# aakhundov/tf-attend-infer-repeat

Measured on AMD Instinct MI355X. Metric: images/sec AIR train step, 50x50 multi-MNIST b=64 N=3, higher is better.
Workload: dtype bf16; 1 GPU; configs[1]: AIR train step, 50x50 canvas, 0-2 objects, batch 64/GPU, 3 steps, 256 LSTM, z=50 (training.py:100-122); global_batch=64, hipgraph=True, steps_per_graph_replay=20, graph_mode=one hipGraph replay = 20 train steps, parallelism=dp1, backward=reference, phase=single order

## Files before the change

include/air_hip.h:

```cpp
#ifndef AIR_HIP_H
#define AIR_HIP_H

#include <stdint.h>

#ifdef __cplusplus
extern "C" {
#endif

#define AIR_ABI_VERSION 6

#define AIR_EINVAL   (-1)
#define AIR_ELIMIT   (-2)
#define AIR_EALIGN   (-3)

int air_abi_version(void);
const char* air_strerror(int code);

enum {
    AIR_DYN_PRIOR_LOG_ODDS = 0,
    AIR_DYN_TEMPERATURE    = 1,
    AIR_DYN_STOP_THRESHOLD = 2,
    AIR_DYN_LEARNING_RATE  = 3,
    AIR_DYN_CLIP_NORM      = 4,
    AIR_DYN_SCALE_PM = 5, AIR_DYN_SCALE_PV = 6,
    AIR_DYN_SHIFT_PM = 7, AIR_DYN_SHIFT_PV = 8,
    AIR_DYN_VAE_PM   = 9, AIR_DYN_VAE_PV   = 10,
    AIR_DYN_LIK_STD  = 11,
    AIR_DYN_GRAD_SCALE = 12,
    AIR_DYN_SCALE_PLV = 13, AIR_DYN_SHIFT_PLV = 14, AIR_DYN_VAE_PLV = 15,
    AIR_DYN_COUNT    = 16
};

enum {
    AIR_IST_GLOBAL_STEP = 0,
    AIR_IST_COUNT = 4
};

typedef struct {
    int32_t slot;
    int32_t flags;
    float init, iters, factor, vmin, vmax;
} air_schedule_t;

enum {
    AIR_ATT_S = 0, AIR_ATT_X = 1, AIR_ATT_Y = 2,
    AIR_ATT_ZPRE = 3,
    AIR_ATT_Z = 4,
    AIR_ATT_ZPROB = 5,
    AIR_ATT_KL_Z = 6, AIR_ATT_KL_SCALE = 7, AIR_ATT_KL_SHIFT = 8, AIR_ATT_KL_VAE = 9,
    AIR_ATT_MASK_PREV = 10,
    AIR_ATT_MASK = 11,
    AIR_ATT_ST_BACK = 12,
    AIR_ATT_STRIDE = 16
};
#define AIR_OUT_STRIDE 8

enum {
    AIR_ACT_NONE = 0, AIR_ACT_RELU = 1, AIR_ACT_SOFTPLUS = 2,
    AIR_ACT_SIGMOID_NOISE = 3
};
enum {
    AIR_GRAD_NONE = 0,
    AIR_GRAD_RELU = 1,
    AIR_GRAD_SOFTPLUS = 2
};
enum {
    AIR_EPI_GENERIC = 0,
    AIR_EPI_LSTM_FWD = 1,
    AIR_EPI_REPARAM_FWD = 2,
    AIR_EPI_LSTM_BWD = 3,
    AIR_EPI_REPARAM_BWD = 4,
    AIR_EPI_LSTM_BWD_TAIL = 5,
    AIR_EPI_LSTM_FWD0 = 6
};
typedef struct {
    const air_schedule_t* sched ; int32_t nsched; float* dyn; const int32_t* istate;
    float* normals; int64_t n_normal; float* uniforms; int64_t n_uniform; uint64_t seed;
    const float* twin_src; uint16_t* twin_dst; int64_t twin_n;
} air_step_job_t;
typedef struct {
    const float* A; const float* B; float* C;
    int32_t M, N, K, lda, ldb, ldc;
    int32_t transA, transB;
    const float* bias;
    const float* addend; int32_t ldadd;
    const float* aux;    int32_t ldaux;
    float   aux_scale;
    int32_t act;
    int32_t actgrad;
    int32_t accumulate;
    int32_t precision;
    int32_t epi;
    int32_t tile_m, tile_n;
    int32_t ksplit;
    int32_t addend_slabs;
    int32_t i0;
    const float* p0; const float* p1; const float* p2; const float* p3;
    float* q0; float* q1; float* q2;
    const air_step_job_t* step_job;
    const uint16_t* A16; const uint16_t* B16;
    uint16_t* C16; uint16_t* q0_16; uint16_t* q2_16;
    const uint16_t* B16p;
} air_gemm_t;
int air_gemm_slabs(int K, int ksplit);
int air_gemm(const air_gemm_t* g, void* stream);
int air_gemm_kernel_name(const air_gemm_t* g, char* buf, int n);

int air_bf16_twin(const float* src, uint16_t* dst, int64_t n, void* stream);

typedef struct {
    int64_t src_off, dst_off;
    int32_t K, N, gates, exclusive;
} air_panel_t;
#define AIR_MAX_PANELS 16
int air_panel_shadow(const float* params, uint16_t* panel_shadow, const air_panel_t* panels ,
                     int count, void* stream);

typedef struct {
    const float* A; const float* dY; float* dW; float* db ;
    int32_t M, N, K, lda, ldb, ldc;
    int32_t head_pack, Hs, Hh, Hz;
    const uint16_t* A16; const uint16_t* dY16;
} air_wgrad_t;
int air_wgrad_num_blocks(const air_wgrad_t* probs, int count);
int air_wgrad_num_workgroups(const air_wgrad_t* probs, int count, int precision);
int air_wgrad_grouped(const air_wgrad_t* probs , int count, int precision,
                      float* sq_partials, int32_t* istate, void* stream);

typedef struct { const float* src; float* dst; int32_t rows, cols, ld, accumulate; } air_colsum_t;
int air_colsum(const air_colsum_t* probs , int count, void* stream);

int air_lstm_gates_fwd(const float* gates_pre, const float* c_prev, float* acts,
                       float* c, float* h, int B, int R, void* stream);
int air_lstm_first_step(const float* xw_slabs, int nslabs, const float* bias , float* acts,
                        float* c, float* h, uint16_t* h16 , int B, int R, void* stream);
int air_lstm_gates_bwd(const float* dh, const float* dc_in , const float* acts,
                       const float* c_prev, const float* c, float* dgates, float* dc_prev,
                       float* dgsum , int dgsum_accumulate, int B, int R, void* stream);

int air_transformer_fwd(const float* U, const float* theta, float* out,
                        int B, int Hi, int Wi, int Ho, int Wo, void* stream);
int air_transformer_bwd(const float* U, const float* theta, const float* d_out, float* d_U, float* d_theta,
                        int B, int Hi, int Wi, int Ho, int Wo, void* stream);

int air_transformer_nc_fwd(const float* U, const float* theta, float* out,
                           int B, int T, int Hi, int Wi, int C, int Ho, int Wo, void* stream);
int air_transformer_nc_bwd(const float* U, const float* theta, const float* d_out,
                           float* d_U , float* d_theta ,
                           int B, int T, int Hi, int Wi, int C, int Ho, int Wo, void* stream);

typedef struct {
    const float* hid; const float* wout; const float* bout;
    const float* canvas;
    const float* eps_scale; const float* eps_shift; const float* u;
    const float* dyn;
    float* out7;
    float* att;
    float* window;
    int32_t B, N, C, w, Hs, Hh, Hz, wout_ld, train;
    uint16_t* window16;
} air_attend_fwd_t;
int air_attend_fwd(const air_attend_fwd_t* a, void* stream);

typedef struct {
    const float* hid; const float* wout;
    const float* canvas; const float* eps_scale; const float* eps_shift;
    const float* dyn; const float* out7; const float* att;
    const float* d_window;
    const float* d_sxy_write;
    float* d_hid;
    float* d_out7;
    int32_t B, N, C, w, Hs, Hh, Hz, wout_ld;
    int32_t literal;
    uint16_t* d_hid16;
} air_attend_bwd_t;
int air_attend_bwd(const air_attend_bwd_t* a, void* stream);

int air_heads_out_wgrad(const float* d_out7, const float* hid, float* dwout, float* dbout,
                        int rows, int Hs, int Hh, int Hz, int wout_ld, void* stream);

int air_reparam_fwd(const float* ml , const float* eps_z, float* zs,
                    int B, int Z, void* stream);
int air_reparam_bwd(const float* d_zs, const float* ml, const float* eps_z, const float* att,
                    const float* dyn, float* d_ml, int B, int Z, void* stream);

typedef struct {
    const float* vrec;
    const float* ml;
    const float* images;
    const float* dyn;
    float* att;
    float* recon;
    float* rec_loss;
    float* d_recon;
    float* run_loss;
    int32_t* run_digits;
    float* loss_item;
    int32_t B, N, C, w, Z;
    int32_t* wb_order;
} air_write_fwd_t;
int air_write_fwd(const air_write_fwd_t* a, void* stream);

typedef struct {
    const float* d_recon;
    const float* vrec; const float* att;
    float* d_gen_pre;
    float* d_sxy_write;
    int32_t B, N, C, w;
    int32_t literal;
    const float* fin_loss_item; const int32_t* fin_targets; const int32_t* fin_digits;
    float* fin_scalars;
    uint16_t* d_gen_pre16;
    const int32_t* order;
} air_write_bwd_t;
int air_write_bwd(const air_write_bwd_t* a, void* stream);
int air_write_bwd_kernel_name(const air_write_bwd_t* a, char* buf, int n);

typedef struct {
    const float* X; const float* Wml; const float* bml; const float* eps; const float* Wg; const float* bg;
    float* ml; float* z; float* g;
    int32_t M, K1, Z, H, ldx;
    uint16_t* z16; uint16_t* g16;
    const uint16_t* X16; const uint16_t* Wml16; const uint16_t* Wg16;
    int32_t exact_fp32;
    int32_t ldz;
} air_bottleneck_fwd_t;
typedef struct {
    const float* dG; const float* Wg; const float* ml; const float* eps;
    const float* att;
    const float* dyn; const float* Wml; const float* x;
    float* d_ml; float* d_x;
    int32_t M, K1, Z, H;
    uint16_t* d_ml16; uint16_t* d_x16;
    const uint16_t* dG16; const uint16_t* Wg16; const uint16_t* Wml16;
    int32_t exact_fp32;
} air_bottleneck_bwd_t;
int air_vae_bottleneck_fwd(const air_bottleneck_fwd_t* a, void* stream);
int air_vae_bottleneck_bwd(const air_bottleneck_bwd_t* a, void* stream);

int air_bce_fwd_bwd(const float* images, const float* run_recon, const float* dyn,
                    float* recon , float* rec_loss ,
                    float* d_recon , int B, int D, void* stream);
int air_finalize(const float* run_loss, const float* rec_loss, const int32_t* targets,
                 const int32_t* digits, float* loss_per_item, float* scalars, int B, void* stream);

int air_step_begin(const air_schedule_t* sched , int nsched, float* dyn,
                   const int32_t* istate, float* normals, int64_t n_normal,
                   float* uniforms, int64_t n_uniform, uint64_t seed,
                   const float* twin_src , uint16_t* twin_dst, int64_t twin_n, void* stream);

int air_optim_num_partials(int64_t n);
int air_grad_sqnorm(const float* grads, int64_t n, float* partials, int32_t* istate, void* stream);
int air_adam_clip_step(float* params, const float* grads, float* m, float* v, int64_t n,
                       const float* partials, int npartials, const float* dyn, const int32_t* istate,
                       float grad_prescale , float beta1, float beta2,
                       float epsilon, uint16_t* bf16_shadow , float* gnorm_out ,
                       void* stream);
int air_adam_clip_step_panels(float* params, const float* grads, float* m, float* v, int64_t n,
                              const float* partials, int npartials, const float* dyn, const int32_t* istate,
                              float grad_prescale, float beta1, float beta2, float epsilon,
                              uint16_t* bf16_shadow , const air_panel_t* panels , int npanels,
                              uint16_t* panel_shadow, float* gnorm_out , void* stream);

typedef struct {
    int32_t* queue;
    int64_t* state;
    int32_t* picks;
    int32_t capacity, batch, min_after_dequeue, n_records;
    uint64_t seed;
} air_shuffle_batch_t;
int air_shuffle_batch_init(const air_shuffle_batch_t* q, void* stream);
int air_shuffle_batch_dequeue(const air_shuffle_batch_t* q, void* stream);
int air_shuffle_batch_dequeue_many(const air_shuffle_batch_t* q, int n_batches, int32_t* picks_out, void* stream);
int air_batch_gather(const float* images, const int32_t* digits, const int32_t* picks, float* out_images,
                     int32_t* out_digits, int batch, int D, void* stream);

#define AIR_MAX_STEPS_SUMMARY 16
typedef struct {
    const float* att;
    const int32_t* targets;
    const int32_t* digits;
    const float* rec_loss;
    const float* loss_item;
    const float* scalars;
    float* out;
    int32_t B, N, max_digits;
} air_summaries_t;
int air_summaries_count(int N, int max_digits);
int air_summaries(const air_summaries_t* a, void* stream);

#define AIR_MAX_STEPS 16
typedef struct {
    const float* scale_src;
    const float* shift_src;
    const float* z_src;
    const float* pres_src;
    const float* dyn;
    float* att;
    float* z;
    uint16_t* z16;
    int32_t B, N, Z, ldz, given;
} air_scene_records_t;
int air_scene_records(const air_scene_records_t* a, void* stream);

typedef struct {
    const float* vrec;
    const float* att;
    float* canvas;
    int32_t* num_digits;
    int32_t B, N, C, w;
} air_render_t;
int air_render(const air_render_t* a, void* stream);

int air_philox_fill(float* normals, int64_t n_normal, float* uniforms, int64_t n_uniform,
                    uint64_t seed, uint64_t call, void* stream);

typedef struct {
    int64_t attend_fwd, attend_bwd, write_fwd, render, write_bwd_exact, write_bwd_graph, limit;
} air_step_lds_t;
int air_step_lds(int N, int C, int w, int Hs, int Hh, int Hz, int wout_ld, air_step_lds_t* out);

typedef struct { const float* ptr; float value; int32_t stride; } air_scalar_t;

int air_concrete_sample_fwd(const float* log_odds, const float* u, const air_scalar_t* temperature, float eps, int hard,
                            float* y , float* sig_y , int64_t n, void* stream);
int air_concrete_sample_bwd(const float* y, const air_scalar_t* temperature, const float* d_y ,
                            const float* d_sig_y , float* d_log_odds, int64_t n, void* stream);
int air_concrete_presigmoid_fwd(const float* log_odds, const float* u, const air_scalar_t* temperature, float eps,
                                float* y, int64_t n, void* stream);
int air_concrete_presigmoid_bwd(const float* d_y, const air_scalar_t* temperature, float* d_log_odds, int64_t n, void* stream);
int air_concrete_kl_fwd(const float* y, const air_scalar_t* prior_log_odds, const air_scalar_t* prior_temperature,
                        const float* posterior_log_odds, const air_scalar_t* posterior_temperature, float eps,
                        float* kl, int64_t n, void* stream);
int air_concrete_kl_bwd(const float* d_kl, const float* y, const air_scalar_t* prior_log_odds,
                        const air_scalar_t* prior_temperature, const float* posterior_log_odds,
                        const air_scalar_t* posterior_temperature, float eps, float* d_y ,
                        float* d_posterior_log_odds , float* d_prior_log_odds , int64_t n, void* stream);

int air_sigmoid_bwd(const float* d_rec, const float* rec, float* d_pre, int64_t n, void* stream);
int air_reparam_bwd_plain(const float* d_z, const float* ml, const float* eps, const float* d_mean_in ,
                          const float* d_lv_in , float* d_ml, int M, int Z, void* stream);

#ifdef __cplusplus
}
#endif
#endif
```

tf-attend-infer-repeat_amd/air/_hip.py:

```python
from __future__ import annotations

import ctypes as C
import os

import torch

_HERE = os.path.dirname(os.path.abspath(__file__))
LIB_PATH = os.environ.get("AIR_HIP_LIB") or os.path.join(os.path.dirname(_HERE), "libair_hip.so")

ABI_VERSION = 6

DYN_PRIOR_LOG_ODDS, DYN_TEMPERATURE, DYN_STOP_THRESHOLD, DYN_LEARNING_RATE, DYN_CLIP_NORM = 0, 1, 2, 3, 4
DYN_SCALE_PM, DYN_SCALE_PV, DYN_SHIFT_PM, DYN_SHIFT_PV, DYN_VAE_PM, DYN_VAE_PV = 5, 6, 7, 8, 9, 10
DYN_LIK_STD, DYN_GRAD_SCALE, DYN_COUNT = 11, 12, 16
DYN_SCALE_PLV, DYN_SHIFT_PLV, DYN_VAE_PLV = 13, 14, 15
IST_GLOBAL_STEP, IST_COUNT = 0, 4
ATT_S, ATT_X, ATT_Y, ATT_ZPRE, ATT_Z, ATT_ZPROB = 0, 1, 2, 3, 4, 5
ATT_KL_Z, ATT_KL_SCALE, ATT_KL_SHIFT, ATT_KL_VAE, ATT_MASK_PREV, ATT_MASK, ATT_ST_BACK = 6, 7, 8, 9, 10, 11, 12
ATT_STRIDE, OUT_STRIDE = 16, 8
ACT_NONE, ACT_RELU, ACT_SOFTPLUS, ACT_SIGMOID_NOISE = 0, 1, 2, 3
GRAD_NONE, GRAD_RELU, GRAD_SOFTPLUS = 0, 1, 2
EPI_GENERIC, EPI_LSTM_FWD, EPI_REPARAM_FWD, EPI_LSTM_BWD, EPI_REPARAM_BWD, EPI_LSTM_BWD_TAIL, EPI_LSTM_FWD0 = 0, 1, 2, 3, 4, 5, 6
SCHED_STAIRCASE, SCHED_HAS_MIN, SCHED_HAS_MAX, SCHED_LOG = 1, 2, 4, 8

_p = C.c_void_p
_i = C.c_int32
_f = C.c_float


class Schedule(C.Structure):
    _fields_ = [("slot", _i), ("flags", _i), ("init", _f), ("iters", _f), ("factor", _f),
                ("vmin", _f), ("vmax", _f)]


class StepJob(C.Structure):
    _fields_ = [("sched", _p), ("nsched", _i), ("dyn", _p), ("istate", _p),
                ("normals", _p), ("n_normal", C.c_int64), ("uniforms", _p), ("n_uniform", C.c_int64),
                ("seed", C.c_uint64), ("twin_src", _p), ("twin_dst", _p), ("twin_n", C.c_int64)]


class Gemm(C.Structure):
    _fields_ = [("A", _p), ("B", _p), ("C", _p),
                ("M", _i), ("N", _i), ("K", _i), ("lda", _i), ("ldb", _i), ("ldc", _i),
                ("transA", _i), ("transB", _i),
                ("bias", _p), ("addend", _p), ("ldadd", _i), ("aux", _p), ("ldaux", _i),
                ("aux_scale", _f), ("act", _i), ("actgrad", _i), ("accumulate", _i), ("precision", _i),
                ("epi", _i), ("tile_m", _i), ("tile_n", _i), ("ksplit", _i), ("addend_slabs", _i), ("i0", _i),
                ("p0", _p), ("p1", _p), ("p2", _p), ("p3", _p), ("q0", _p), ("q1", _p), ("q2", _p),
                ("step_job", C.POINTER(StepJob)),
                ("A16", _p), ("B16", _p), ("C16", _p), ("q0_16", _p), ("q2_16", _p), ("B16p", _p)]


class Panel(C.Structure):
    _fields_ = [("src_off", C.c_int64), ("dst_off", C.c_int64), ("K", _i), ("N", _i), ("gates", _i), ("exclusive", _i)]


MAX_PANELS = 16


class Colsum(C.Structure):
    _fields_ = [("src", _p), ("dst", _p), ("rows", _i), ("cols", _i), ("ld", _i), ("accumulate", _i)]


class Wgrad(C.Structure):
    _fields_ = [("A", _p), ("dY", _p), ("dW", _p), ("db", _p),
                ("M", _i), ("N", _i), ("K", _i), ("lda", _i), ("ldb", _i), ("ldc", _i),
                ("head_pack", _i), ("Hs", _i), ("Hh", _i), ("Hz", _i), ("A16", _p), ("dY16", _p)]


class AttendFwd(C.Structure):
    _fields_ = [("hid", _p), ("wout", _p), ("bout", _p), ("canvas", _p),
                ("eps_scale", _p), ("eps_shift", _p), ("u", _p), ("dyn", _p),
                ("out7", _p), ("att", _p), ("window", _p),
                ("B", _i), ("N", _i), ("C", _i), ("w", _i), ("Hs", _i), ("Hh", _i), ("Hz", _i),
                ("wout_ld", _i), ("train", _i), ("window16", _p)]


class AttendBwd(C.Structure):
    _fields_ = [("hid", _p), ("wout", _p), ("canvas", _p), ("eps_scale", _p), ("eps_shift", _p),
                ("dyn", _p), ("out7", _p), ("att", _p), ("d_window", _p), ("d_sxy_write", _p),
                ("d_hid", _p), ("d_out7", _p),
                ("B", _i), ("N", _i), ("C", _i), ("w", _i), ("Hs", _i), ("Hh", _i), ("Hz", _i), ("wout_ld", _i),
                ("literal", _i), ("d_hid16", _p)]


class WriteFwd(C.Structure):
    _fields_ = [("vrec", _p), ("ml", _p), ("images", _p), ("dyn", _p), ("att", _p), ("recon", _p),
                ("rec_loss", _p), ("d_recon", _p), ("run_loss", _p), ("run_digits", _p), ("loss_item", _p),
                ("B", _i), ("N", _i), ("C", _i), ("w", _i), ("Z", _i), ("wb_order", _p)]


class WriteBwd(C.Structure):
    _fields_ = [("d_recon", _p), ("vrec", _p), ("att", _p), ("d_gen_pre", _p), ("d_sxy_write", _p),
                ("B", _i), ("N", _i), ("C", _i), ("w", _i), ("literal", _i),
                ("fin_loss_item", _p), ("fin_targets", _p), ("fin_digits", _p), ("fin_scalars", _p), ("d_gen_pre16", _p),
                ("order", _p)]


class BottleneckFwd(C.Structure):
    _fields_ = [("X", _p), ("Wml", _p), ("bml", _p), ("eps", _p), ("Wg", _p), ("bg", _p), ("ml", _p), ("z", _p), ("g", _p),
                ("M", _i), ("K1", _i), ("Z", _i), ("H", _i), ("ldx", _i), ("z16", _p), ("g16", _p),
                ("X16", _p), ("Wml16", _p), ("Wg16", _p), ("exact_fp32", _i), ("ldz", _i)]


class BottleneckBwd(C.Structure):
    _fields_ = [("dG", _p), ("Wg", _p), ("ml", _p), ("eps", _p), ("att", _p), ("dyn", _p), ("Wml", _p), ("x", _p),
                ("d_ml", _p), ("d_x", _p), ("M", _i), ("K1", _i), ("Z", _i), ("H", _i), ("d_ml16", _p), ("d_x16", _p),
                ("dG16", _p), ("Wg16", _p), ("Wml16", _p), ("exact_fp32", _i)]


class ShuffleBatch(C.Structure):
    _fields_ = [("queue", _p), ("state", _p), ("picks", _p), ("capacity", _i), ("batch", _i), ("min_after_dequeue", _i),
                ("n_records", _i), ("seed", C.c_uint64)]


class Summaries(C.Structure):
    _fields_ = [("att", _p), ("targets", _p), ("digits", _p), ("rec_loss", _p), ("loss_item", _p), ("scalars", _p),
                ("out", _p), ("B", _i), ("N", _i), ("max_digits", _i)]


class SceneRecords(C.Structure):
    _fields_ = [("scale_src", _p), ("shift_src", _p), ("z_src", _p), ("pres_src", _p), ("dyn", _p), ("att", _p),
                ("z", _p), ("z16", _p), ("B", _i), ("N", _i), ("Z", _i), ("ldz", _i), ("given", _i)]


class Render(C.Structure):
    _fields_ = [("vrec", _p), ("att", _p), ("canvas", _p), ("num_digits", _p), ("B", _i), ("N", _i), ("C", _i), ("w", _i)]


MAX_STEPS = 16


class StepLds(C.Structure):
    _fields_ = [(k, C.c_int64) for k in ("attend_fwd", "attend_bwd", "write_fwd", "render", "write_bwd_exact",
                                         "write_bwd_graph", "limit")]


class Scalar(C.Structure):
    _fields_ = [("ptr", _p), ("value", _f), ("stride", _i)]


_SIGNATURES = {
    "air_abi_version": (C.c_int, []),
    "air_strerror": (C.c_char_p, [C.c_int]),
    "air_gemm": (C.c_int, [C.POINTER(Gemm), _p]),
    "air_gemm_kernel_name": (C.c_int, [C.POINTER(Gemm), C.c_char_p, C.c_int]),
    "air_gemm_slabs": (C.c_int, [C.c_int, C.c_int]),
    "air_bf16_twin": (C.c_int, [_p, _p, C.c_int64, _p]),
    "air_panel_shadow": (C.c_int, [_p, _p, C.POINTER(Panel), C.c_int, _p]),
    "air_adam_clip_step_panels": (C.c_int, [_p, _p, _p, _p, C.c_int64, _p, C.c_int, _p, _p, _f, _f, _f, _f, _p,
                                            C.POINTER(Panel), C.c_int, _p, _p, _p]),
    "air_colsum": (C.c_int, [C.POINTER(Colsum), C.c_int, _p]),
    "air_wgrad_num_blocks": (C.c_int, [C.POINTER(Wgrad), C.c_int]),
    "air_wgrad_num_workgroups": (C.c_int, [C.POINTER(Wgrad), C.c_int, C.c_int]),
    "air_wgrad_grouped": (C.c_int, [C.POINTER(Wgrad), C.c_int, C.c_int, _p, _p, _p]),
    "air_lstm_gates_fwd": (C.c_int, [_p, _p, _p, _p, _p, C.c_int, C.c_int, _p]),
    "air_lstm_first_step": (C.c_int, [_p, C.c_int, _p, _p, _p, _p, _p, C.c_int, C.c_int, _p]),
    "air_lstm_gates_bwd": (C.c_int, [_p, _p, _p, _p, _p, _p, _p, _p, C.c_int, C.c_int, C.c_int, _p]),
    "air_transformer_fwd": (C.c_int, [_p, _p, _p, C.c_int, C.c_int, C.c_int, C.c_int, C.c_int, _p]),
    "air_transformer_bwd": (C.c_int, [_p, _p, _p, _p, _p, C.c_int, C.c_int, C.c_int, C.c_int, C.c_int, _p]),
    "air_transformer_nc_fwd": (C.c_int, [_p, _p, _p] + [C.c_int] * 7 + [_p]),
    "air_transformer_nc_bwd": (C.c_int, [_p, _p, _p, _p, _p] + [C.c_int] * 7 + [_p]),
    "air_attend_fwd": (C.c_int, [C.POINTER(AttendFwd), _p]),
    "air_attend_bwd": (C.c_int, [C.POINTER(AttendBwd), _p]),
    "air_heads_out_wgrad": (C.c_int, [_p, _p, _p, _p, C.c_int, C.c_int, C.c_int, C.c_int, C.c_int, _p]),
    "air_reparam_fwd": (C.c_int, [_p, _p, _p, C.c_int, C.c_int, _p]),
    "air_reparam_bwd": (C.c_int, [_p, _p, _p, _p, _p, _p, C.c_int, C.c_int, _p]),
    "air_write_fwd": (C.c_int, [C.POINTER(WriteFwd), _p]),
    "air_write_bwd": (C.c_int, [C.POINTER(WriteBwd), _p]),
    "air_bce_fwd_bwd": (C.c_int, [_p, _p, _p, _p, _p, _p, C.c_int, C.c_int, _p]),
    "air_finalize": (C.c_int, [_p, _p, _p, _p, _p, _p, C.c_int, _p]),
    "air_step_begin": (C.c_int, [_p, C.c_int, _p, _p, _p, C.c_int64, _p, C.c_int64, C.c_uint64, _p, _p, C.c_int64, _p]),
    "air_optim_num_partials": (C.c_int, [C.c_int64]),
    "air_grad_sqnorm": (C.c_int, [_p, C.c_int64, _p, _p, _p]),
    "air_write_bwd_kernel_name": (C.c_int, [C.POINTER(WriteBwd), C.c_char_p, C.c_int]),
    "air_vae_bottleneck_fwd": (C.c_int, [C.POINTER(BottleneckFwd), _p]),
    "air_vae_bottleneck_bwd": (C.c_int, [C.POINTER(BottleneckBwd), _p]),
    "air_adam_clip_step": (C.c_int, [_p, _p, _p, _p, C.c_int64, _p, C.c_int, _p, _p, _f, _f, _f, _f, _p, _p, _p]),
    "air_shuffle_batch_init": (C.c_int, [C.POINTER(ShuffleBatch), _p]),
    "air_shuffle_batch_dequeue": (C.c_int, [C.POINTER(ShuffleBatch), _p]),
    "air_shuffle_batch_dequeue_many": (C.c_int, [C.POINTER(ShuffleBatch), C.c_int, _p, _p]),
    "air_batch_gather": (C.c_int, [_p, _p, _p, _p, _p, C.c_int, C.c_int, _p]),
    "air_summaries_count": (C.c_int, [C.c_int, C.c_int]),
    "air_summaries": (C.c_int, [C.POINTER(Summaries), _p]),
    "air_scene_records": (C.c_int, [C.POINTER(SceneRecords), _p]),
    "air_render": (C.c_int, [C.POINTER(Render), _p]),
    "air_philox_fill": (C.c_int, [_p, C.c_int64, _p, C.c_int64, C.c_uint64, C.c_uint64, _p]),
    "air_step_lds": (C.c_int, [C.c_int] * 7 + [C.POINTER(StepLds)]),
    "air_concrete_sample_fwd": (C.c_int, [_p, _p, C.POINTER(Scalar), _f, C.c_int, _p, _p, C.c_int64, _p]),
    "air_concrete_sample_bwd": (C.c_int, [_p, C.POINTER(Scalar), _p, _p, _p, C.c_int64, _p]),
    "air_concrete_presigmoid_fwd": (C.c_int, [_p, _p, C.POINTER(Scalar), _f, _p, C.c_int64, _p]),
    "air_concrete_presigmoid_bwd": (C.c_int, [_p, C.POINTER(Scalar), _p, C.c_int64, _p]),
    "air_concrete_kl_fwd": (C.c_int, [_p, C.POINTER(Scalar), C.POINTER(Scalar), _p, C.POINTER(Scalar), _f, _p, C.c_int64, _p]),
    "air_concrete_kl_bwd": (C.c_int, [_p, _p, C.POINTER(Scalar), C.POINTER(Scalar), _p, C.POINTER(Scalar), _f, _p, _p, _p,
                                      C.c_int64, _p]),
    "air_sigmoid_bwd": (C.c_int, [_p, _p, _p, C.c_int64, _p]),
    "air_reparam_bwd_plain": (C.c_int, [_p, _p, _p, _p, _p, _p, C.c_int, C.c_int, _p]),
}

EXPORTED_SYMBOLS = tuple(_SIGNATURES)


class AirHipError(RuntimeError):
    pass


def load(path: str = LIB_PATH):
    if not os.path.exists(path):
        raise AirHipError(
            "libair_hip.so not found at %s -- the AIR hot path has no CPU fallback. "
            "Build it: python tf-attend-infer-repeat_amd/build.py" % path)
    lib = C.CDLL(path)
    for name, (res, args) in _SIGNATURES.items():
        try:
            fn = getattr(lib, name)
        except AttributeError as e:
            raise AirHipError("libair_hip.so lacks symbol %s (stale build?)" % name) from e
        fn.restype = res
        fn.argtypes = args
    if lib.air_abi_version() != ABI_VERSION:
        raise AirHipError("libair_hip.so ABI %d != binding ABI %d" % (lib.air_abi_version(), ABI_VERSION))
    return lib


_LIB = None


def lib():
    global _LIB
    if _LIB is None:
        _LIB = load()
    return _LIB


def check(rc: int, what: str = ""):
    if rc != 0:
        msg = lib().air_strerror(rc)
        raise AirHipError("%s failed with code %d: %s" % (what or "libair_hip call", rc,
                                                          msg.decode() if msg else "?"))
```

tf-attend-infer-repeat_amd/csrc/air_gemm.hip:

```cpp
#include "air_gemm_common.h"
#include <cstdlib>
#include <type_traits>
#include <cstdio>

AIR_STAMPS_READER(air_debug_stamps_gemm)

using namespace airg;

namespace {

template <int TM, int TN, bool TA, bool TB>
__global__ __launch_bounds__(THREADS) void gemm_f32_kernel(Args a)
{
    constexpr int EPI_ = -1;
    constexpr int BM = 16 * TM, BN = 16 * TN;
    constexpr int BKC = (TM * TN >= 4) ? 64 : 128;
    constexpr int LA = TA ? (BM == 16 ? 16 : BM + 16) : BM + 1;
    constexpr int LB = TB ? BN + 1 : (BN == 16 ? 16 : BN + 16);
    constexpr int PA = BM * BKC / 1024, PB = BN * BKC / 1024;
    constexpr int NCHR = 32 / (PA + PB);
    constexpr int NCH = NCHR < 1 ? 1 : (NCHR > 8 ? 8 : NCHR);
    __shared__ __attribute__((aligned(16))) float As[2][BKC * LA];
    __shared__ __attribute__((aligned(16))) float Bs[2][BKC * LB];
    __shared__ float Red[3 * TM * TN * 4 * 64];

    if ((int)blockIdx.z < a.job_on) {
        const long plane = (long)gridDim.x * gridDim.y;
        air_step_job_run(a.job, blockIdx.z * plane + (long)blockIdx.y * gridDim.x + blockIdx.x, plane * a.job_on);
        return;
    }
    const int nslab = (int)gridDim.z - a.job_on;
    const int zslab = (int)blockIdx.z - a.job_on;
    const int tid = threadIdx.x, lane = tid & 63, wave = tid >> 6;
    int tile_m, tile_n;
    xcd_tile(tile_m, tile_n);
    const int m0 = tile_m * BM, n0 = tile_n * BN / TN * (a.gstride == 16 ? TN : 1);
    const int kbeg = zslab * a.kslab;
    const int kend = min(a.K, kbeg + a.kslab);

    f32x4 acc[TM][TN];
#pragma unroll
    for (int i = 0; i < TM; ++i)
#pragma unroll
        for (int j = 0; j < TN; ++j) acc[i][j] = f32x4{0.f, 0.f, 0.f, 0.f};

    const bool vecA = ((a.lda & 3) == 0) && aligned16(a.A);
    const bool vecB = ((a.ldb & 3) == 0) && aligned16(a.B) && ((a.gstride & 3) == 0);
    Pre<TM, TN> pre;
    if (nslab == 1) epilogue_prefetch<TM, TN, EPI_>(a, pre, m0, n0, lane, wave);

    auto loadA = [&](int k0, int i) -> float4 {
        float4 v = make_float4(0.f, 0.f, 0.f, 0.f);
        if (!TA) {
            const int g = wave + 4 * i;
            const int m = (g % (BM / 4)) * 4 + (lane & 3);
            const int k4 = (g / (BM / 4)) * 16 + (lane >> 2);
            const int gm = m0 + m, gk = k0 + k4 * 4;
            if (gm < a.M && gk < kend) {
                const float* src = a.A + (size_t)gm * a.lda + gk;
                if (vecA && gk + 3 < kend) v = *reinterpret_cast<const float4*>(src);
                else {
                    v.x = src[0];
                    if (gk + 1 < kend) v.y = src[1];
                    if (gk + 2 < kend) v.z = src[2];
                    if (gk + 3 < kend) v.w = src[3];
                }
            }
        } else {
            constexpr int MQ = BM / 4;
            const int it = tid + THREADS * i;
            const int k = it / MQ, mq = it % MQ;
            const int gm = m0 + mq * 4, gk = k0 + k;
            if (gk < kend && gm < a.M) {
                const float* src = a.A + (size_t)gk * a.lda + gm;
                if (vecA && gm + 3 < a.M) v = *reinterpret_cast<const float4*>(src);
                else {
                    v.x = src[0];
                    if (gm + 1 < a.M) v.y = src[1];
                    if (gm + 2 < a.M) v.z = src[2];
                    if (gm + 3 < a.M) v.w = src[3];
                }
            }
        }
        return v;
    };
    auto storeA = [&](float* as, int i, const float4& v) {
        if (!TA) {
            const int g = wave + 4 * i;
            const int m = (g % (BM / 4)) * 4 + (lane & 3);
            const int k4 = (g / (BM / 4)) * 16 + (lane >> 2);
            float* d = as + (size_t)(k4 * 4) * LA + m;
            d[0] = v.x; d[LA] = v.y; d[2 * LA] = v.z; d[3 * LA] = v.w;
        } else {
            constexpr int MQ = BM / 4;
            const int it = tid + THREADS * i;
            *reinterpret_cast<float4*>(as + (size_t)(it / MQ) * LA + (it % MQ) * 4) = v;
        }
    };
    auto loadB = [&](int k0, int i) -> float4 {
        float4 v = make_float4(0.f, 0.f, 0.f, 0.f);
        if (TB) {
            const int g = wave + 4 * i;
            const int n = (g % (BN / 4)) * 4 + (lane & 3);
            const int k4 = (g / (BN / 4)) * 16 + (lane >> 2);
            const int gn = n0 + n, gk = k0 + k4 * 4;
            if (gn < a.N && gk < kend) {
                const float* src = a.B + (size_t)gn * a.ldb + gk;
                if (vecB && gk + 3 < kend) v = *reinterpret_cast<const float4*>(src);
                else {
                    v.x = src[0];
                    if (gk + 1 < kend) v.y = src[1];
                    if (gk + 2 < kend) v.z = src[2];
                    if (gk + 3 < kend) v.w = src[3];
                }
            }
        } else {
            constexpr int NQ = BN / 4;
            const int it = tid + THREADS * i;
            const int k = it / NQ, q4 = it % NQ;
            const int j = q4 >> 2, c = (q4 & 3) * 4;
            const int cg = n0 + c + (a.gstride == 16 ? j * 16 : 0);
            const int gn = n0 + j * a.gstride + c, gk = k0 + k;
            if (gk < kend) {
                const float* src = a.B + (size_t)gk * a.ldb + gn;
                const int lim = min(a.gwidth - cg, a.N - gn);
                if (vecB && lim >= 4) v = *reinterpret_cast<const float4*>(src);
                else {
                    if (lim > 0) v.x = src[0];
                    if (lim > 1) v.y = src[1];
                    if (lim > 2) v.z = src[2];
                    if (lim > 3) v.w = src[3];
                }
            }
        }
        return v;
    };
    auto storeB = [&](float* bs, int i, const float4& v) {
        if (TB) {
            const int g = wave + 4 * i;
            const int n = (g % (BN / 4)) * 4 + (lane & 3);
            const int k4 = (g / (BN / 4)) * 16 + (lane >> 2);
            float* d = bs + (size_t)(k4 * 4) * LB + n;
            d[0] = v.x; d[LB] = v.y; d[2 * LB] = v.z; d[3 * LB] = v.w;
        } else {
            constexpr int NQ = BN / 4;
            const int it = tid + THREADS * i;
            *reinterpret_cast<float4*>(bs + (size_t)(it / NQ) * LB + (it % NQ) * 4) = v;
        }
    };

    for (int ks0 = kbeg; ks0 < kend; ks0 += NCH * BKC) {
        if (ks0 > kbeg) __syncthreads();
        float4 va[NCH][PA], vb[NCH][PB];
#pragma unroll
        for (int c = 0; c < NCH; ++c) {
            const int k0 = ks0 + c * BKC;
            if (k0 < kend) {
#pragma unroll
                for (int i = 0; i < PA; ++i) va[c][i] = loadA(k0, i);
#pragma unroll
                for (int i = 0; i < PB; ++i) vb[c][i] = loadB(k0, i);
            }
        }
#pragma unroll
        for (int c = 0; c < NCH; ++c) {
            const int k0 = ks0 + c * BKC;
            if (k0 < kend) {
                float* as = As[c & 1];
                float* bs = Bs[c & 1];
#pragma unroll
                for (int i = 0; i < PA; ++i) storeA(as, i, va[c][i]);
#pragma unroll
                for (int i = 0; i < PB; ++i) storeB(bs, i, vb[c][i]);
                __syncthreads();
                const int steps = (min(BKC, kend - k0) + 3) >> 2;
                constexpr int SU = BKC / 16;
                float av[SU][TM], bv[SU][TN];
#pragma unroll
                for (int u = 0; u < SU; ++u) {
                    const int sidx = wave + 4 * u;
                    const bool ok = sidx < steps;
                    const int kk = (ok ? sidx : 0) * 4 + (lane >> 4);
#pragma unroll
                    for (int i = 0; i < TM; ++i) { const float t = as[(size_t)kk * LA + i * 16 + (lane & 15)]; av[u][i] = ok ? t : 0.0f; }
#pragma unroll
                    for (int j = 0; j < TN; ++j) { const float t = bs[(size_t)kk * LB + j * 16 + (lane & 15)]; bv[u][j] = ok ? t : 0.0f; }
                }
#pragma unroll
                for (int u = 0; u < SU; ++u)
#pragma unroll
                    for (int i = 0; i < TM; ++i)
#pragma unroll
                        for (int j = 0; j < TN; ++j)
                            acc[i][j] = __builtin_amdgcn_mfma_f32_16x16x4f32(av[u][i], bv[u][j], acc[i][j], 0, 0, 0);
            }
        }
    }
    reduce_waves<TM, TN>(acc, Red, lane, wave);
    if (nslab > 1) {
        float* Cz = a.C + (size_t)zslab * a.slab_stride;
        for (int t = wave; t < TM * TN; t += 4) {
            const int i = t / TN, j = t % TN;
#pragma unroll
            for (int q = 0; q < 4; ++q) {
                const int m = m0 + i * 16 + (lane >> 4) * 4 + q;
                const int n = n0 + j * 16 + (lane & 15);
                if (m < a.M && n < a.N) Cz[(size_t)m * a.ldc + n] = Red[(t * 4 + q) * 64 + lane];
            }
        }
        return;
    }
    epilogue<TM, TN, EPI_>(a, pre, Red, m0, n0, lane, wave);
}

template <int TM, int TN, bool TA, bool TB>
__global__ __launch_bounds__(THREADS) void gemm_bf16_kernel(Args a)
{
    constexpr int BK = 128;
    constexpr int BM = 16 * TM, BN = 16 * TN;
    constexpr int LK = BK + 8;
    constexpr int NA = BM * BK / THREADS;
    constexpr int NB = BN * BK / THREADS;
    __shared__ __attribute__((aligned(16))) unsigned short As[BM * LK];
    __shared__ __attribute__((aligned(16))) unsigned short Bs[BN * LK];
    __shared__ float Red[3 * TM * TN * 4 * 64];

    if ((int)blockIdx.z < a.job_on) {
        const long plane = (long)gridDim.x * gridDim.y;
        air_step_job_run(a.job, blockIdx.z * plane + (long)blockIdx.y * gridDim.x + blockIdx.x, plane * a.job_on);
        return;
    }
    const int nslab = (int)gridDim.z - a.job_on;
    const int zslab = (int)blockIdx.z - a.job_on;
    const int tid = threadIdx.x, lane = tid & 63, wave = tid >> 6;
    int tile_m, tile_n;
    xcd_tile(tile_m, tile_n);
    const int m0 = tile_m * BM, n0 = tile_n * BN / TN * (a.gstride == 16 ? TN : 1);
    const int kbeg = zslab * a.kslab;
    const int kend = min(a.K, kbeg + a.kslab);

    float ra[NA], rb[NB];
    auto fetch = [&](int k0) {
#pragma unroll
        for (int i = 0; i < NA; ++i) {
            const int idx = tid + i * THREADS;
            int m, k;
            if (TA) { k = idx / BM; m = idx % BM; } else { m = idx / BK; k = idx % BK; }
            const int gm = m0 + m, gk = k0 + k;
            float v = 0.0f;
            if (gm < a.M && gk < kend) v = TA ? a.A[(size_t)gk * a.lda + gm] : a.A[(size_t)gm * a.lda + gk];
            ra[i] = v;
        }
#pragma unroll
        for (int i = 0; i < NB; ++i) {
            const int idx = tid + i * THREADS;
            int n, k;
            if (TB) { n = idx / BK; k = idx % BK; } else { k = idx / BN; n = idx % BN; }
            const int j = n >> 4, c = n & 15;
            const int cg = n0 + c + (a.gstride == 16 ? j * 16 : 0);
            const int gn = n0 + j * a.gstride + c, gk = k0 + k;
            float v = 0.0f;
            if (cg < a.gwidth && gn < a.N && gk < kend)
                v = TB ? a.B[(size_t)gn * a.ldb + gk] : a.B[(size_t)gk * a.ldb + gn];
            rb[i] = v;
        }
    };
    auto stage = [&]() {
#pragma unroll
        for (int i = 0; i < NA; ++i) {
            const int idx = tid + i * THREADS;
            int m, k;
            if (TA) { k = idx / BM; m = idx % BM; } else { m = idx / BK; k = idx % BK; }
            As[m * LK + k] = f32_to_bf16_rne(ra[i]);
        }
#pragma unroll
        for (int i = 0; i < NB; ++i) {
            const int idx = tid + i * THREADS;
            int n, k;
            if (TB) { n = idx / BK; k = idx % BK; } else { k = idx / BN; n = idx % BN; }
            Bs[n * LK + k] = f32_to_bf16_rne(rb[i]);
        }
    };

    f32x4 acc[TM][TN];
#pragma unroll
    for (int i = 0; i < TM; ++i)
#pragma unroll
        for (int j = 0; j < TN; ++j) acc[i][j] = f32x4{0.f, 0.f, 0.f, 0.f};

    fetch(kbeg);
    for (int k0 = kbeg; k0 < kend; k0 += BK) {
        __syncthreads();
        stage();
        __syncthreads();
        if (k0 + BK < kend) fetch(k0 + BK);
        const int kk = wave * 32 + (lane >> 4) * 8;
        bf16x8 av[TM], bv[TN];
#pragma unroll
        for (int i = 0; i < TM; ++i) av[i] = *reinterpret_cast<const bf16x8*>(&As[(i * 16 + (lane & 15)) * LK + kk]);
#pragma unroll
        for (int j = 0; j < TN; ++j) bv[j] = *reinterpret_cast<const bf16x8*>(&Bs[(j * 16 + (lane & 15)) * LK + kk]);
#pragma unroll
        for (int i = 0; i < TM; ++i)
#pragma unroll
            for (int j = 0; j < TN; ++j)
                acc[i][j] = __builtin_amdgcn_mfma_f32_16x16x32_bf16(av[i], bv[j], acc[i][j], 0, 0, 0);
    }
    reduce_waves<TM, TN>(acc, Red, lane, wave);
    if (nslab > 1) {
        float* Cz = a.C + (size_t)zslab * a.slab_stride;
        for (int t = wave; t < TM * TN; t += 4) {
            const int i = t / TN, j = t % TN;
#pragma unroll
            for (int q = 0; q < 4; ++q) {
                const int m = m0 + i * 16 + (lane >> 4) * 4 + q;
                const int n = n0 + j * 16 + (lane & 15);
                if (m < a.M && n < a.N) Cz[(size_t)m * a.ldc + n] = Red[(t * 4 + q) * 64 + lane];
            }
        }
        return;
    }
    Pre<TM, TN> pre;
    epilogue_prefetch<TM, TN, -1>(a, pre, m0, n0, lane, wave);
    epilogue<TM, TN, -1>(a, pre, Red, m0, n0, lane, wave);
}


__device__ __forceinline__ float4 ldg16(const char* base, unsigned off, bool ok) {
    const uint4 t = *reinterpret_cast<const uint4*>(base + (ok ? off : 0u));
    const unsigned m = ok ? 0xffffffffu : 0u;
    return make_float4(__uint_as_float(t.x & m), __uint_as_float(t.y & m), __uint_as_float(t.z & m), __uint_as_float(t.w & m));
}

__device__ __forceinline__ float2 ldg8(const char* base, unsigned off, bool ok) {
    const uint2 t = *reinterpret_cast<const uint2*>(base + (ok ? off : 0u));
    const unsigned m = ok ? 0xffffffffu : 0u;
    return make_float2(__uint_as_float(t.x & m), __uint_as_float(t.y & m));
}
template <bool HALF>
__device__ __forceinline__ float4 ldg16x(const char* base, unsigned off, bool ok_lo, bool ok_hi) {
    if (!HALF) return ldg16(base, off, ok_lo);
    const float2 lo = ldg8(base, off, ok_lo), hi = ldg8(base, off + 8u, ok_hi);
    return make_float4(lo.x, lo.y, hi.x, hi.y);
}

template <int TM, int TN>
struct V2Cfg {
    static constexpr int BM = 16 * TM, BN = 16 * TN, KB = 64;
    static constexpr int IMG = (BM + BN) * KB;
    static constexpr int RL = 49152 / (IMG * 2);
    static constexpr int RV = 28 / (TM + TN);
    static constexpr int R0 = RL < RV ? RL : RV;
    static constexpr int R = R0 > 8 ? 8 : (R0 < 1 ? 1 : R0);
    static constexpr int RED = 3 * TM * TN * 4 * 64 * 4;
    static constexpr int BYTES = (R * IMG * 2 > RED) ? R * IMG * 2 : RED;
};

template <int TM, int TN, bool TB, int EPI_>
__global__ __launch_bounds__(THREADS) void gemm_bf16v2_kernel(Args a)
{
    using Cfg = V2Cfg<TM, TN>;
    constexpr int BM = Cfg::BM, BN = Cfg::BN, KB = Cfg::KB, R = Cfg::R;
    __shared__ __attribute__((aligned(16))) unsigned char Lds[Cfg::BYTES];
    unsigned short* ImgA = reinterpret_cast<unsigned short*>(Lds);
    unsigned short* ImgB = ImgA + R * BM * KB;
    float* Red = reinterpret_cast<float*>(Lds);

    if ((int)blockIdx.z < a.job_on) {
        const long plane = (long)gridDim.x * gridDim.y;
        air_step_job_run(a.job, blockIdx.z * plane + (long)blockIdx.y * gridDim.x + blockIdx.x, plane * a.job_on);
        return;
    }
    const int nslab = (int)gridDim.z - a.job_on;
    const int zslab = (int)blockIdx.z - a.job_on;
    const int tid = threadIdx.x, lane = tid & 63, wave = tid >> 6;
    int tile_m, tile_n;
    xcd_tile(tile_m, tile_n);
    const int m0 = tile_m * BM, n0 = EPI_ == AIR_EPI_LSTM_FWD0 ? tile_n * 4 : tile_n * BN / TN * (a.gstride == 16 ? TN : 1);
    const int kbeg = zslab * a.kslab;
    const int kend = min(a.K, kbeg + a.kslab);

    AIR_STAMP(56);
    f32x4 acc[TM][TN];
#pragma unroll
    for (int i = 0; i < TM; ++i)
#pragma unroll
        for (int j = 0; j < TN; ++j) acc[i][j] = f32x4{0.f, 0.f, 0.f, 0.f};

    Pre<TM, TN> pre;

    const char* Ab = reinterpret_cast<const char*>(a.A);
    const char* Bb = reinterpret_cast<const char*>(a.B);
    const bool a8 = !(((a.lda & 3) == 0) && aligned16(a.A) && ((a.K & 3) == 0));
    const bool b8 = !(((a.ldb & 3) == 0) && aligned16(a.B) &&
                      (TB ? ((a.K & 3) == 0) : (((a.N & 3) == 0) && ((a.gstride & 3) == 0) && ((a.gwidth & 3) == 0))));
    constexpr int TA_N = (R * BM * 8 + THREADS - 1) / THREADS;
    constexpr int TBK_N = (R * BN * 8 + THREADS - 1) / THREADS;
    constexpr int TBN_N = (R * BN * 2 + THREADS - 1) / THREADS;

    float4 va[TA_N][2];
    float4 vbk[TB ? TBK_N : 1][2];
    float4 vbn[TB ? 1 : TBN_N][8];
    auto issue_loads_t = [&](int kr, auto ha_t, auto hb_t) __attribute__((always_inline)) {
        constexpr bool HA = decltype(ha_t)::value, HB = decltype(hb_t)::value;
#pragma unroll
        for (int i = 0; i < 2 * TA_N; ++i) {
            const int u = tid + THREADS * i;
            const int c = u / (BM * 16), row = (u / 16) % BM, hh = u & 15;
            const int gm = m0 + row, gk = kr + c * KB + hh * 4;
            const bool okr = (u < R * BM * 16) && gm < a.M;
            const unsigned off = ((unsigned)gm * (unsigned)a.lda + (unsigned)gk) * 4u;
            va[i >> 1][i & 1] = ldg16x<HA>(Ab, off, okr && gk < kend, okr && gk + 2 < kend);
        }
        if (TB) {
#pragma unroll
            for (int i = 0; i < 2 * TBK_N; ++i) {
                const int u = tid + THREADS * i;
                const int c = u / (BN * 16), col = (u / 16) % BN, hh = u & 15;
                const int j = col >> 4, cc = col & 15;
                const int gn = n0 + j * a.gstride + cc, cg = n0 + cc + (a.gstride == 16 ? j * 16 : 0);
                const int gk = kr + c * KB + hh * 4;
                const bool okr = (u < R * BN * 16) && cg < a.gwidth && gn < a.N;
                const unsigned off = ((unsigned)gn * (unsigned)a.ldb + (unsigned)gk) * 4u;
                vbk[i >> 1][i & 1] = ldg16x<HB>(Bb, off, okr && gk < kend, okr && gk + 2 < kend);
            }
        } else {
#pragma unroll
            for (int i = 0; i < TBN_N; ++i) {
                const int t = tid + THREADS * i;
                const int c = t / (BN * 2), q = (t / 8) % (BN / 4), g = t & 7;
                const int col = q * 4, j = col >> 4, cc = col & 15;
                const int gn = EPI_ == AIR_EPI_LSTM_FWD0 ? n0 + q * a.gstride : n0 + j * a.gstride + cc;
                const int cg = EPI_ == AIR_EPI_LSTM_FWD0 ? n0 : n0 + cc + (a.gstride == 16 ? j * 16 : 0);
                const int gk = kr + c * KB + g * 8;
                const bool okc = (t < R * BN * 2) && cg < a.gwidth && gn < a.N;
                const bool okh = okc && cg + 2 < a.gwidth && gn + 2 < a.N;
                const unsigned off = ((unsigned)gk * (unsigned)a.ldb + (unsigned)gn) * 4u;
#pragma unroll
                for (int r = 0; r < 8; ++r)
                    vbn[i][r] = ldg16x<HB>(Bb, off + (unsigned)r * ((unsigned)a.ldb * 4u), okc && gk + r < kend,
                                           okh && gk + r < kend);
            }
        }
    };
    auto k_loop = [&](auto ha_t, auto hb_t) __attribute__((always_inline)) {
    auto issue_loads = [&](int kr) __attribute__((always_inline)) { issue_loads_t(kr, ha_t, hb_t); };
    issue_loads(kbeg);
    if (nslab == 1) epilogue_prefetch<TM, TN, EPI_>(a, pre, m0, n0, lane, wave);
    AIR_STAMP(57);
    for (int kr = kbeg; kr < kend; kr += R * KB) {
        if (kr > kbeg) __syncthreads();
#pragma unroll
        for (int i = 0; i < 2 * TA_N; ++i) {
            const int u = tid + THREADS * i;
            const int c = u / (BM * 16), row = (u / 16) % BM, hh = u & 15;
            const float4& x = va[i >> 1][i & 1];
            uint2 w;
            w.x = air_pack_bf16(x.x, x.y); w.y = air_pack_bf16(x.z, x.w);
            if (u < R * BM * 16)
                *reinterpret_cast<uint2*>(&ImgA[(c * BM + row) * KB + (((hh >> 1) ^ (row & 7)) << 3) + (hh & 1) * 4]) = w;
        }
        if (TB) {
#pragma unroll
            for (int i = 0; i < 2 * TBK_N; ++i) {
                const int u = tid + THREADS * i;
                const int c = u / (BN * 16), col = (u / 16) % BN, hh = u & 15;
                const float4& x = vbk[i >> 1][i & 1];
                uint2 w;
                w.x = air_pack_bf16(x.x, x.y); w.y = air_pack_bf16(x.z, x.w);
                if (u < R * BN * 16)
                    *reinterpret_cast<uint2*>(&ImgB[(c * BN + col) * KB + (((hh >> 1) ^ (col & 7)) << 3) + (hh & 1) * 4]) = w;
            }
        } else {
#pragma unroll
            for (int i = 0; i < TBN_N; ++i) {
                const int t = tid + THREADS * i;
                const int c = t / (BN * 2), q = (t / 8) % (BN / 4), g = t & 7;
                if (t < R * BN * 2) {
#pragma unroll
                    for (int e = 0; e < 4; ++e) {
                        const int col = q * 4 + e;
                        auto el = [&](int r) { const float4& x = vbn[i][r]; return e == 0 ? x.x : e == 1 ? x.y : e == 2 ? x.z : x.w; };
                        uint4 w;
                        w.x = air_pack_bf16(el(0), el(1)); w.y = air_pack_bf16(el(2), el(3));
                        w.z = air_pack_bf16(el(4), el(5)); w.w = air_pack_bf16(el(6), el(7));
                        *reinterpret_cast<uint4*>(&ImgB[(c * BN + col) * KB + ((g ^ (col & 7)) << 3)]) = w;
                    }
                }
            }
        }
        if (kr + R * KB < kend) issue_loads(kr + R * KB);
        __syncthreads();
        AIR_STAMP(58);
        const int cfirst = (wave - ((kr - kbeg) / KB)) & 3;
#pragma unroll
        for (int cc = 0; cc < (R + 3) / 4; ++cc) {
            const int c = cfirst + 4 * cc;
            if (c < R && kr + c * KB < kend) {
#pragma unroll
                for (int ks = 0; ks < 2; ++ks) {
                    const int slot = ks * 4 + (lane >> 4);
                    bf16x8 av[TM], bv[TN];
#pragma unroll
                    for (int i = 0; i < TM; ++i) {
                        const int row = i * 16 + (lane & 15);
                        av[i] = *reinterpret_cast<const bf16x8*>(&ImgA[(c * BM + row) * KB + ((slot ^ (row & 7)) << 3)]);
                    }
#pragma unroll
                    for (int j = 0; j < TN; ++j) {
                        const int col = j * 16 + (lane & 15);
                        bv[j] = *reinterpret_cast<const bf16x8*>(&ImgB[(c * BN + col) * KB + ((slot ^ (col & 7)) << 3)]);
                    }
#pragma unroll
                    for (int i = 0; i < TM; ++i)
#pragma unroll
                        for (int j = 0; j < TN; ++j)
                            acc[i][j] = __builtin_amdgcn_mfma_f32_16x16x32_bf16(av[i], bv[j], acc[i][j], 0, 0, 0);
                }
            }
        }
    }
    };
    {
        using T_ = std::true_type; using F_ = std::false_type;
        if (!a8 && !b8) k_loop(F_{}, F_{});
        else if (!a8) k_loop(F_{}, T_{});
        else if (!b8) k_loop(T_{}, F_{});
        else k_loop(T_{}, T_{});
    }
    AIR_STAMP(59);
    __syncthreads();
    reduce_waves<TM, TN>(acc, Red, lane, wave);
    AIR_STAMP(60);
    if (nslab > 1) {
        float* Cz = a.C + (size_t)zslab * a.slab_stride;
        for (int t = wave; t < TM * TN; t += 4) {
            const int i = t / TN, j = t % TN;
#pragma unroll
            for (int q = 0; q < 4; ++q) {
                const int m = m0 + i * 16 + (lane >> 4) * 4 + q;
                const int n = n0 + j * 16 + (lane & 15);
                if (m < a.M && n < a.N) Cz[(size_t)m * a.ldc + n] = Red[(t * 4 + q) * 64 + lane];
            }
        }
        return;
    }
    epilogue<TM, TN, EPI_>(a, pre, Red, m0, n0, lane, wave);
    AIR_STAMP(61);
}



template <int TM, int TN>
struct F32V2Cfg {
    static constexpr int BM = 16 * TM, BN = 16 * TN, KB = 64;
    static constexpr int IMG = (BM + BN) * KB * 4;
    static constexpr int RL = 81920 / IMG;
    static constexpr int RV = 24 / (TM + TN);
    static constexpr int R0 = RL < RV ? RL : RV;
    static constexpr int R = R0 > 8 ? 8 : (R0 < 1 ? 1 : R0);
    static constexpr int RED = 3 * TM * TN * 4 * 64 * 4;
    static constexpr int BYTES = (R * IMG > RED) ? R * IMG : RED;
};

template <int TM, int TN, bool TB, int EPI_>
__global__ __launch_bounds__(THREADS) void gemm_f32v2_kernel(Args a)
{
    using Cfg = F32V2Cfg<TM, TN>;
    constexpr int BM = Cfg::BM, BN = Cfg::BN, KB = Cfg::KB, R = Cfg::R;
    extern __shared__ __attribute__((aligned(16))) unsigned char Lds[];
    float* ImgA = reinterpret_cast<float*>(Lds);
    float* ImgB = ImgA + R * BM * KB;
    float* Red = reinterpret_cast<float*>(Lds);

    if ((int)blockIdx.z < a.job_on) {
        const long plane = (long)gridDim.x * gridDim.y;
        air_step_job_run(a.job, blockIdx.z * plane + (long)blockIdx.y * gridDim.x + blockIdx.x, plane * a.job_on);
        return;
    }
    const int nslab = (int)gridDim.z - a.job_on;
    const int zslab = (int)blockIdx.z - a.job_on;
    const int tid = threadIdx.x, lane = tid & 63, wave = tid >> 6;
    int tile_m, tile_n;
    xcd_tile(tile_m, tile_n);
    constexpr bool QUADF = EPI_ == AIR_EPI_LSTM_FWD0 || EPI_ == EPI_LSTM_FWD_Q;
    const int m0 = tile_m * BM, n0 = QUADF ? tile_n * 4 : tile_n * BN / TN * (a.gstride == 16 ? TN : 1);
    const int kbeg = zslab * a.kslab;
    const int kend = min(a.K, kbeg + a.kslab);

    f32x4 acc[TM][TN];
#pragma unroll
    for (int i = 0; i < TM; ++i)
#pragma unroll
        for (int j = 0; j < TN; ++j) acc[i][j] = f32x4{0.f, 0.f, 0.f, 0.f};

    Pre<TM, TN> pre;
    if (nslab == 1) epilogue_prefetch<TM, TN, EPI_>(a, pre, m0, n0, lane, wave);

    const char* Ab = reinterpret_cast<const char*>(a.A);
    const char* Bb = reinterpret_cast<const char*>(a.B);
    const bool a8 = !(((a.lda & 3) == 0) && aligned16(a.A) && ((a.K & 3) == 0));
    const bool b8 = !(((a.ldb & 3) == 0) && aligned16(a.B) &&
                      (TB ? ((a.K & 3) == 0) : (((a.N & 3) == 0) && ((a.gstride & 3) == 0) && ((a.gwidth & 3) == 0))));
    constexpr int TA_N = (R * BM * 8 + THREADS - 1) / THREADS;
    constexpr int TBK_N = (R * BN * 8 + THREADS - 1) / THREADS;
    constexpr int TBN_N = (R * BN * 2 + THREADS - 1) / THREADS;

    float4 va[TA_N][2];
    float4 vbk[TB ? TBK_N : 1][2];
    float4 vbn[TB ? 1 : TBN_N][8];
    auto issue_loads_t = [&](int kr, auto ha_t, auto hb_t) __attribute__((always_inline)) {
        constexpr bool HA = decltype(ha_t)::value, HB = decltype(hb_t)::value;
#pragma unroll
        for (int i = 0; i < TA_N; ++i) {
            const int t = tid + THREADS * i;
            const int c = t / (BM * 8), row = (t / 8) % BM, g = t & 7;
            const int gm = m0 + row, gk = kr + c * KB + g * 8;
            const bool okr = (t < R * BM * 8) && gm < a.M;
            const unsigned off = ((unsigned)gm * (unsigned)a.lda + (unsigned)gk) * 4u;
            va[i][0] = ldg16x<HA>(Ab, off, okr && gk < kend, okr && gk + 2 < kend);
            va[i][1] = ldg16x<HA>(Ab, off + 16u, okr && gk + 4 < kend, okr && gk + 6 < kend);
        }
        if (TB) {
#pragma unroll
            for (int i = 0; i < TBK_N; ++i) {
                const int t = tid + THREADS * i;
                const int c = t / (BN * 8), col = (t / 8) % BN, g = t & 7;
                const int j = col >> 4, cc = col & 15;
                const int gn = n0 + j * a.gstride + cc, cg = n0 + cc + (a.gstride == 16 ? j * 16 : 0);
                const int gk = kr + c * KB + g * 8;
                const bool okr = (t < R * BN * 8) && cg < a.gwidth && gn < a.N;
                const unsigned off = ((unsigned)gn * (unsigned)a.ldb + (unsigned)gk) * 4u;
                vbk[i][0] = ldg16x<HB>(Bb, off, okr && gk < kend, okr && gk + 2 < kend);
                vbk[i][1] = ldg16x<HB>(Bb, off + 16u, okr && gk + 4 < kend, okr && gk + 6 < kend);
            }
        } else {
#pragma unroll
            for (int i = 0; i < TBN_N; ++i) {
                const int t = tid + THREADS * i;
                const int c = t / (BN * 2), q = (t / 8) % (BN / 4), g = t & 7;
                const int col = q * 4, j = col >> 4, cc = col & 15;
                const int gn = QUADF ? n0 + q * a.gstride : n0 + j * a.gstride + cc;
                const int cg = QUADF ? n0 : n0 + cc + (a.gstride == 16 ? j * 16 : 0);
                const int gk = kr + c * KB + g * 8;
                const bool okc = (t < R * BN * 2) && cg < a.gwidth && gn < a.N;
                const bool okh = okc && cg + 2 < a.gwidth && gn + 2 < a.N;
                const unsigned off = ((unsigned)gk * (unsigned)a.ldb + (unsigned)gn) * 4u;
#pragma unroll
                for (int r = 0; r < 8; ++r)
                    vbn[i][r] = ldg16x<HB>(Bb, off + (unsigned)r * ((unsigned)a.ldb * 4u), okc && gk + r < kend,
                                       okh && gk + r < kend);
            }
        }
    };
    auto issue_loads = [&](int kr) __attribute__((always_inline)) {
        using T_ = std::true_type; using F_ = std::false_type;
        if (!a8 && !b8) issue_loads_t(kr, F_{}, F_{});
        else if (!a8) issue_loads_t(kr, F_{}, T_{});
        else if (!b8) issue_loads_t(kr, T_{}, F_{});
        else issue_loads_t(kr, T_{}, T_{});
    };
    for (int kr = kbeg; kr < kend; kr += R * KB) {
        if (kr > kbeg) __syncthreads();
        issue_loads(kr);
#pragma unroll
        for (int i = 0; i < TA_N; ++i) {
            const int t = tid + THREADS * i;
            const int c = t / (BM * 8), row = (t / 8) % BM, g = t & 7;
            if (t < R * BM * 8) {
                float* dst = &ImgA[(c * BM + row) * KB];
                *reinterpret_cast<float4*>(dst + (((2 * g) ^ (row & 15)) << 2)) = va[i][0];
                *reinterpret_cast<float4*>(dst + (((2 * g + 1) ^ (row & 15)) << 2)) = va[i][1];
            }
        }
        if (TB) {
#pragma unroll
            for (int i = 0; i < TBK_N; ++i) {
                const int t = tid + THREADS * i;
                const int c = t / (BN * 8), col = (t / 8) % BN, g = t & 7;
                if (t < R * BN * 8) {
                    float* dst = &ImgB[(c * BN + col) * KB];
                    *reinterpret_cast<float4*>(dst + (((2 * g) ^ (col & 15)) << 2)) = vbk[i][0];
                    *reinterpret_cast<float4*>(dst + (((2 * g + 1) ^ (col & 15)) << 2)) = vbk[i][1];
                }
            }
        } else {
#pragma unroll
            for (int i = 0; i < TBN_N; ++i) {
                const int t = tid + THREADS * i;
                const int c = t / (BN * 2), q = (t / 8) % (BN / 4), g = t & 7;
                if (t < R * BN * 2) {
#pragma unroll
                    for (int e = 0; e < 4; ++e) {
                        const int col = q * 4 + e;
                        auto el = [&](int r) { const float4& x = vbn[i][r]; return e == 0 ? x.x : e == 1 ? x.y : e == 2 ? x.z : x.w; };
                        float* dst = &ImgB[(c * BN + col) * KB];
                        *reinterpret_cast<float4*>(dst + (((2 * g) ^ (col & 15)) << 2)) = make_float4(el(0), el(1), el(2), el(3));
                        *reinterpret_cast<float4*>(dst + (((2 * g + 1) ^ (col & 15)) << 2)) = make_float4(el(4), el(5), el(6), el(7));
                    }
                }
            }
        }
        __syncthreads();
#pragma unroll
        for (int cc = 0; cc < (R + 3) / 4; ++cc) {
            const int c = wave + 4 * cc;
            if (c < R && kr + c * KB < kend) {
#pragma unroll
                for (int kb = 0; kb < 4; ++kb) {
                    const int slot = kb * 4 + (lane >> 4);
                    float4 av[TM], bv[TN];
#pragma unroll
                    for (int i = 0; i < TM; ++i) {
                        const int row = i * 16 + (lane & 15);
                        av[i] = *reinterpret_cast<const float4*>(&ImgA[(c * BM + row) * KB + ((slot ^ (row & 15)) << 2)]);
                    }
#pragma unroll
                    for (int j = 0; j < TN; ++j) {
                        const int col = j * 16 + (lane & 15);
                        bv[j] = *reinterpret_cast<const float4*>(&ImgB[(c * BN + col) * KB + ((slot ^ (col & 15)) << 2)]);
                    }
#pragma unroll
                    for (int e = 0; e < 4; ++e)
#pragma unroll
                        for (int i = 0; i < TM; ++i)
#pragma unroll
                            for (int j = 0; j < TN; ++j) {
                                const float ae = e == 0 ? av[i].x : e == 1 ? av[i].y : e == 2 ? av[i].z : av[i].w;
                                const float be = e == 0 ? bv[j].x : e == 1 ? bv[j].y : e == 2 ? bv[j].z : bv[j].w;
                                acc[i][j] = __builtin_amdgcn_mfma_f32_16x16x4f32(ae, be, acc[i][j], 0, 0, 0);
                            }
                }
            }
        }
    }
    __syncthreads();
    reduce_waves<TM, TN>(acc, Red, lane, wave);
    if (nslab > 1) {
        float* Cz = a.C + (size_t)zslab * a.slab_stride;
        for (int t = wave; t < TM * TN; t += 4) {
            const int i = t / TN, j = t % TN;
#pragma unroll
            for (int q = 0; q < 4; ++q) {
                const int m = m0 + i * 16 + (lane >> 4) * 4 + q;
                const int n = n0 + j * 16 + (lane & 15);
                if (m < a.M && n < a.N) Cz[(size_t)m * a.ldc + n] = Red[(t * 4 + q) * 64 + lane];
            }
        }
        return;
    }
    epilogue<TM, TN, EPI_>(a, pre, Red, m0, n0, lane, wave);
}


#define FB(KERNEL, F, TM, TN, TA, TB) {{F, TM, TN, TA, TB, -1, false, 0}, reinterpret_cast<const void*>(&KERNEL<TM, TN, TA, TB>), 0}
#define FB3(KERNEL, F, TM, TN) FB(KERNEL, F, TM, TN, false, false), FB(KERNEL, F, TM, TN, true, false), FB(KERNEL, F, TM, TN, false, true)
#define F32V2_(TM, TN, TB, EPI) \
    {{F32V2, TM, TN, false, TB, EPI, false, 0}, reinterpret_cast<const void*>(&gemm_f32v2_kernel<TM, TN, TB, EPI>), F32V2Cfg<TM, TN>::BYTES}
#define V2(TM, TN, TB, EPI) \
    {{BF16V2, TM, TN, false, TB, EPI, false, 0}, reinterpret_cast<const void*>(&gemm_bf16v2_kernel<TM, TN, TB, EPI>), 0}, F32V2_(TM, TN, TB, EPI)
#define TILE(TM, TN) \
    FB3(gemm_f32_kernel, F32, TM, TN), FB3(gemm_bf16_kernel, BF16, TM, TN), V2(TM, TN, false, AIR_EPI_GENERIC), V2(TM, TN, true, AIR_EPI_GENERIC)
const Kern KERNELS[] = {
    TILE(1, 1), TILE(1, 2), TILE(1, 4), TILE(2, 2), TILE(2, 4), TILE(4, 1), TILE(4, 2), TILE(4, 4),
    V2(1, 4, false, AIR_EPI_LSTM_FWD), V2(1, 2, false, AIR_EPI_REPARAM_FWD), V2(1, 1, false, AIR_EPI_LSTM_FWD0),
    V2(1, 1, false, AIR_EPI_LSTM_BWD), V2(1, 1, false, AIR_EPI_LSTM_BWD_TAIL), V2(1, 1, false, AIR_EPI_REPARAM_BWD),
    V2(1, 1, true, AIR_EPI_LSTM_BWD), V2(1, 1, true, AIR_EPI_LSTM_BWD_TAIL), V2(1, 1, true, AIR_EPI_REPARAM_BWD),
    F32V2_(1, 1, false, EPI_LSTM_FWD_Q)};
#undef TILE
#undef V2
#undef F32V2_
#undef FB3
#undef FB
template <int N> constexpr int count_of(const Kern (&)[N]) { return N; }

const Kern* find_kernel(const Inst& inst) {
    int n = count_of(KERNELS);
    const Kern* k = KERNELS;
    if (inst.family == BF16TW || inst.family == XWX_GLDS || inst.family == XW_TP) k = twin_kernels(n);
    for (int i = 0; i < n; ++i)
        if (k[i].inst == inst) return k + i;
    return nullptr;
}

void resolve_tile(const air_gemm_t* g, int& tm, int& tn) {
    tm = g->tile_m; tn = g->tile_n;
    if (g->epi == AIR_EPI_LSTM_FWD) { tm = 1; tn = 4; }
    else if (g->epi == AIR_EPI_REPARAM_FWD) { tm = 1; tn = 2; }
    else if (g->epi == AIR_EPI_LSTM_FWD0) { tm = 1; tn = 1; }
    else if (g->epi != AIR_EPI_GENERIC) { tm = 1; tn = 1; }
    if (tm == 0 || tn == 0) {
        const long t11 = (long)((g->M + 15) / 16) * ((g->N + 15) / 16);
        if (t11 <= 1024) { tm = 1; tn = 1; }
        else if (t11 <= 4096) { tm = 2; tn = 2; }
        else { tm = 2; tn = 4; }
    }
}

bool use_bf16_v2(const Args& a, bool ta, bool tb) {
    auto al8 = [](const void* p) { return (reinterpret_cast<uintptr_t>(p) & 7) == 0; };
    return !ta && al8(a.A) && al8(a.B) && (a.lda & 1) == 0 && (a.ldb & 1) == 0 && (a.K & 1) == 0 &&
           (tb || ((a.N & 1) == 0 && (a.gstride & 1) == 0 && (a.gwidth & 1) == 0));
}

int kslab_of(int K, int ksplit) {
    const int ks = ksplit > 1 ? ksplit : 1;
    return ((K + ks - 1) / ks + 3) & ~3;
}

int job_planes(const Args& a, dim3 grid, int cap) {
    if (!a.job_on) return 0;
    const long quads = (a.job.n_normal + 3) / 4 + (a.job.n_uniform + 3) / 4 + (a.job.twin_n + 3) / 4;
    const long plane = (long)grid.x * grid.y * THREADS;
    const long planes = (quads + plane - 1) / plane;
    return (int)(planes < 1 ? 1 : (planes > cap ? cap : planes));
}

int images_of(const Args& a) { return (a.kslab + 63) / 64; }

bool fwd0_padded(const Args& a) { return a.epi == AIR_EPI_LSTM_FWD0 && a.A16 != nullptr && (a.i0 & 2) != 0; }
bool fwd0_glds(const Args& a) { return fwd0_padded(a) && (a.i0 & 1) == 0; }

int twin_rounds(const Args& a, int tm, int tn, bool ta, bool tb) {
    const bool pnl_tile = !tb && a.B16p != nullptr && ((tm == 1 && tn == 1) || (tm == 2 && tn == 2) || (tm == 1 && tn == 4));
    if (ta || (!a.B16 && !pnl_tile)) return 0;
    auto al16 = [](const void* p) { return (reinterpret_cast<uintptr_t>(p) & 15) == 0; };
    const bool af32 = a.A16 == nullptr;
    const bool padded = fwd0_padded(a);
    if (af32) { if (!al16(a.A) || (a.lda & 3) || (a.K & 3) || (a.kslab & 3) || (a.epi == AIR_EPI_LSTM_FWD0 && !al16(a.C16))) return 0; }
    else if (padded) { if (!al16(a.A16) || (a.lda & 7) || a.lda < ((a.K + 7) & ~7) || !pnl_tile || tb) return 0; }
    else if (!al16(a.A16) || (a.lda & 7) || (a.K & 7) || (a.kslab & 7)) return 0;
    if (pnl_tile) { if (!al16(a.B16p)) return 0; }
    else if (!al16(a.B16) || (a.ldb & 7)) return 0;
    if (tb) { if ((a.K & 7) || (a.kslab & 7)) return 0; }
    else if ((a.N & 7) || (a.gstride & 7) || (a.gwidth & 7)) return 0;
    const int nimg = images_of(a);
    const int e = a.epi;
    if (tm == 1 && tn == 1) {
        if (e == AIR_EPI_LSTM_FWD0)
            return (!tb && (a.gwidth & 3) == 0 && (int)((a.K + a.kslab - 1) / a.kslab) == 1)
                       ? ((nimg <= 40 && nimg > 16) ? 40 : 16) : 0;
        if (af32) return 0;
        if (e == AIR_EPI_GENERIC || ((e == AIR_EPI_LSTM_BWD || e == AIR_EPI_LSTM_BWD_TAIL) && tb)) return nimg <= 4 ? 4 : (nimg <= 8 ? 8 : 16);
        return 0;
    }
    if (tm == 1 && tn == 4) return (!af32 && !tb && e == AIR_EPI_LSTM_FWD) ? 4 : 0;
    if (tm == 2 && tn == 2) return e == AIR_EPI_GENERIC ? (af32 ? (tb ? 0 : 8) : (nimg <= 4 ? 4 : 8)) : 0;
    if (tm == 4 && tn == 2) return (e == AIR_EPI_GENERIC && !tb) ? 4 : 0;
    if (tm == 4 && tn == 4) return (e == AIR_EPI_GENERIC && !tb) ? 4 : 0;
    return 0;
}

int xw_tp_ok(const Args& a, int precision, bool ta, bool tb, int ksplit) {
    auto al16 = [](const void* p) { return (reinterpret_cast<uintptr_t>(p) & 15) == 0; };
    if (precision != 1 || ta || tb || !a.B16 || a.epi != AIR_EPI_GENERIC || ksplit <= 1) return AIR_EINVAL;
    if ((a.M % 64) || (a.N % 64) || (a.kslab % 64) || (a.K % 64)) return AIR_EALIGN;
    if (!al16(a.A) || !al16(a.B16) || (a.lda & 3) || (a.ldb & 7)) return AIR_EALIGN;
    return 0;
}

int xw_tp_columns(const Args& a) {
    const long slabs = (a.K + a.kslab - 1) / a.kslab;
    const bool wide = (a.N % 128) == 0 && (long)(a.N / 128) * (a.M / 64) * slabs >= 256;
    return wide ? 128 : 64;
}

}

int airg::plan_gemm(const air_gemm_t* g, const Args& filled, Plan& p) {
    Args& a = p.args;
    a = filled;
    a.kslab = kslab_of(a.K, g->ksplit);
    a.slab_stride = (long)a.M * a.ldc;
    const bool ta = g->transA != 0, tb = g->transB != 0;
    if (g->tile_m == 8 && g->tile_n == 4) {
        const int ok = xw_tp_ok(a, g->precision, ta, tb, g->ksplit);
        if (ok) return ok;
        const int cols = xw_tp_columns(a);
        p.inst = Inst{XW_TP, 8, 4, false, false, AIR_EPI_GENERIC, false, cols};
        p.grid = dim3(a.N / cols, a.M / 64, 1);
        a.job_on = job_planes(a, p.grid, 64);
    } else {
        int tm, tn;
        resolve_tile(g, tm, tn);
        if (!find_kernel(Inst{F32, tm, tn, false, false, -1, false, 0})) return AIR_EINVAL;
        const bool grouped = a.gstride != 16;
        const int ncols = grouped ? a.gwidth : a.N;
        const int tile_cols = a.epi == AIR_EPI_LSTM_FWD0 ? 4 : (grouped ? 16 : 16 * tn);
        p.grid = dim3((ncols + tile_cols - 1) / tile_cols, (a.M + 16 * tm - 1) / (16 * tm), 1);
        a.job_on = job_planes(a, p.grid, 16);
        const int r = g->precision == 1 ? twin_rounds(a, tm, tn, ta, tb) : 0;
        const bool lean = use_bf16_v2(a, ta, tb);
        bool quad = false;
        if (r > 0) {
            p.inst = Inst{fwd0_glds(a) ? XWX_GLDS : BF16TW, tm, tn, false, tb, a.epi, a.A16 == nullptr, r};
            quad = tm == 1 && tn == 4;
        } else {
            if (a.epi == AIR_EPI_LSTM_FWD0 && (a.C16 || fwd0_padded(a) || !lean)) return AIR_EALIGN;
            if (lean) p.inst = Inst{g->precision == 1 ? BF16V2 : F32V2, tm, tn, false, tb, a.epi, false, 0};
            else p.inst = Inst{g->precision == 1 ? BF16 : F32, tm, tn, ta, tb, -1, false, 0};
            quad = lean && g->precision == 0 && a.epi == AIR_EPI_LSTM_FWD && (a.gwidth & 3) == 0 && !a.job_on;
        }
        if (quad) {
            p.inst.tn = 1;
            p.inst.epi = EPI_LSTM_FWD_Q;
            const unsigned wide = p.grid.x;
            p.grid.x = (a.gwidth + 3) / 4;
            if (a.job_on) a.job_on = (int)((a.job_on * wide + p.grid.x - 1) / p.grid.x);
        }
    }
    p.grid.z = (a.K + a.kslab - 1) / a.kslab + a.job_on;
    const Kern* k = find_kernel(p.inst);
    if (!k) return AIR_EINVAL;
    if ((size_t)k->lds > AIR_LDS_LIMIT) return AIR_ELIMIT;
    p.fn = k->fn;
    p.lds = k->lds;
    return 0;
}

extern "C" int air_gemm_slabs(int K, int ksplit) {
    if (K <= 0) return 0;
    const int kslab = kslab_of(K, ksplit);
    return (K + kslab - 1) / kslab;
}

static int fill_args(const air_gemm_t* g, Args& a);

extern "C" int air_gemm(const air_gemm_t* g, void* stream) {
    Args a;
    Plan p;
    int rc = fill_args(g, a);
    if (!rc) rc = plan_gemm(g, a, p);
    if (rc) return rc;
    if (p.inst.family == F32V2 && p.lds > 48 * 1024)
        for (const Kern& k : KERNELS) {
            const Inst& i = k.inst;
            const bool variant = i.family == F32V2 && i.tm == p.inst.tm && i.tn == p.inst.tn && i.tb == p.inst.tb &&
                                 (i.epi == EPI_LSTM_FWD_Q) == (p.inst.epi == EPI_LSTM_FWD_Q);
            if (variant && (rc = air_grant_lds(k.fn, k.lds)) != 0) return rc;
        }
    else if ((rc = air_grant_lds(p.fn, p.lds)) != 0) return rc;
    void* kargs[] = {&p.args};
    (void)hipLaunchKernel(p.fn, p.grid, dim3(THREADS), kargs, p.lds, air_stream(stream));
    AIR_CHECK_LAUNCH();
    return 0;
}

extern "C" int air_gemm_kernel_name(const air_gemm_t* g, char* buf, int n) {
    Args a;
    Plan p;
    int rc = fill_args(g, a);
    if (rc) return rc;
    if (!buf || n <= 0) return AIR_EINVAL;
    if ((rc = plan_gemm(g, a, p)) != 0) return rc;
    static const char* const FAMILY[] = {"f32", "bf16", "f32v2", "bf16v2", "bf16tw", "xwx_glds", "xw_tp"};
    const Inst& i = p.inst;
    auto tf = [](bool b) { return b ? "true" : "false"; };
    const char* fam = FAMILY[i.family];
    switch (i.family) {
        case F32: case BF16: snprintf(buf, n, "gemm_%s_kernel<%d, %d, %s, %s>", fam, i.tm, i.tn, tf(i.ta), tf(i.tb)); break;
        case F32V2: case BF16V2: snprintf(buf, n, "gemm_%s_kernel<%d, %d, %s, %d>", fam, i.tm, i.tn, tf(i.tb), i.epi); break;
        case BF16TW: snprintf(buf, n, "gemm_%s_kernel<%d, %d, %s, %d, %s, %d>", fam, i.tm, i.tn, tf(i.tb), i.epi, tf(i.af32), i.r); break;
        default: snprintf(buf, n, "gemm_%s_kernel<%d>", fam, i.r); break;
    }
    return 0;
}

static int fill_args(const air_gemm_t* g, Args& a) {
    if (!g || !g->A || !g->B || !g->C) return AIR_EINVAL;
    if (g->M <= 0 || g->N <= 0 || g->K <= 0) return AIR_EINVAL;
    if (g->precision != 0 && g->precision != 1) return AIR_EINVAL;
    if ((g->act == AIR_ACT_SIGMOID_NOISE || g->actgrad != AIR_GRAD_NONE) && !g->aux) return AIR_EINVAL;
    if (g->transA && g->transB) return AIR_EINVAL;
    if (g->epi < AIR_EPI_GENERIC || g->epi > AIR_EPI_LSTM_FWD0) return AIR_EINVAL;
    if (g->ksplit > 1 && g->epi != AIR_EPI_GENERIC) return AIR_EINVAL;
    if (g->addend_slabs > 8) return AIR_ELIMIT;
    const bool lda_is_twins = g->epi == AIR_EPI_LSTM_FWD0 && g->A16 && (g->i0 & 2);
    if (!lda_is_twins && g->lda < (g->transA ? g->M : g->K)) return AIR_EINVAL;
    if (g->ldb < (g->transB ? g->K : g->N)) return AIR_EINVAL;
    if (g->ldc < (g->epi == AIR_EPI_REPARAM_BWD ? 2 * g->N : g->N)) return AIR_EINVAL;
    if (g->addend && g->ldadd < g->N) return AIR_EINVAL;
    if (g->aux && g->ldaux < g->N) return AIR_EINVAL;
    a.A = g->A; a.B = g->B; a.C = g->C;
    a.M = g->M; a.N = g->N; a.K = g->K; a.lda = g->lda; a.ldb = g->ldb; a.ldc = g->ldc;
    a.gstride = 16; a.gwidth = g->N;
    a.kslab = g->K; a.slab_stride = 0;
    a.bias = g->bias; a.addend = g->addend; a.aux = g->aux;
    a.ldadd = g->ldadd; a.ldaux = g->ldaux;
    a.add_slabs = g->addend ? (g->addend_slabs > 0 ? g->addend_slabs : 1) : 0;
    a.add_slab_stride = (long)g->M * g->ldadd;
    a.aux_scale = g->aux_scale;
    a.act = g->act; a.actgrad = g->actgrad; a.accumulate = g->accumulate; a.epi = g->epi;
    a.p0 = g->p0; a.p1 = g->p1; a.p2 = g->p2; a.p3 = g->p3; a.p4 = nullptr;
    a.q0 = g->q0; a.q1 = g->q1; a.q2 = g->q2; a.q3 = nullptr;
    a.i0 = g->i0; a.i1 = 0;
    a.A16 = g->A16; a.B16 = g->B16; a.C16 = g->C16; a.q0_16 = g->q0_16; a.q2_16 = g->q2_16;
    a.B16p = (g->precision == 1 && !g->transA && !g->transB) ? g->B16p : nullptr;
    a.job_on = 0;
    if (g->step_job) {
        const air_step_job_t& j = *g->step_job;
        if (!j.dyn || !j.istate || j.nsched < 0 || j.nsched > THREADS || (j.nsched > 0 && !j.sched)) return AIR_EINVAL;
        if (j.n_normal < 0 || j.n_uniform < 0 || (j.n_normal > 0 && !j.normals) || (j.n_uniform > 0 && !j.uniforms)) return AIR_EINVAL;
        a.job_on = 1;
        if (j.twin_n < 0 || (j.twin_n > 0 && (!j.twin_src || !j.twin_dst))) return AIR_EINVAL;
        if (j.twin_n > 0 && (!aligned16(j.twin_src) || (reinterpret_cast<uintptr_t>(j.twin_dst) & 7) != 0)) return AIR_EALIGN;
        a.job = AirStepJob{j.sched, j.nsched, j.dyn, j.istate, j.normals, (long)j.n_normal, j.uniforms, (long)j.n_uniform,
                           (uint32_t)(j.seed & 0xffffffffu), (uint32_t)(j.seed >> 32), j.twin_src, j.twin_dst, (long)j.twin_n};
    }
    switch (g->epi) {
        case AIR_EPI_LSTM_FWD:
            if (g->transA || g->transB || (g->N & 3) || !g->p0 || !g->q0 || !g->q1 || !g->q2) return AIR_EINVAL;
            a.gstride = g->N / 4; a.gwidth = g->N / 4; break;
        case AIR_EPI_LSTM_FWD0:
            if (g->transA || g->transB || (g->N & 15) || g->addend || !g->q0 || !g->q1 || !g->q2) return AIR_EINVAL;
            a.gstride = g->N / 4; a.gwidth = g->N / 4; break;
        case AIR_EPI_REPARAM_FWD:
            if (g->transA || g->transB || (g->N & 1) || !g->p0 || !g->q0) return AIR_EINVAL;
            a.gstride = g->N / 2; a.gwidth = g->N / 2; break;
        case AIR_EPI_LSTM_BWD:
            if (!g->p0 || !g->p1 || !g->p2 || !g->q0 || !g->q1) return AIR_EINVAL;
            a.gwidth = g->N; break;
        case AIR_EPI_LSTM_BWD_TAIL:
            if (!g->p0 || !g->p1 || !g->p2 || !g->q0 || !g->q1 || g->p3 || g->i0 < 0 || g->i0 > g->M) return AIR_EINVAL;
            a.gwidth = g->N; break;
        case AIR_EPI_REPARAM_BWD:
            if (!g->p0 || !g->p1 || !g->p2 || !g->p3) return AIR_EINVAL;
            a.gwidth = g->N; break;
        default: break;
    }
    return 0;
}
```

tf-attend-infer-repeat_amd/csrc/air_gemm_bf16.hip:

```cpp
#include "air_gemm_common.h"
#include <atomic>
#include <cstdlib>
#include <cstdio>

using namespace airg;

AIR_STAMPS_READER(air_debug_stamps_gemm_tw)

namespace {

typedef short s16x4 __attribute__((ext_vector_type(4)));

__device__ __forceinline__ uint4 ldg16u(const char* base, unsigned off, bool ok) {
    const uint4 t = *reinterpret_cast<const uint4*>(base + (ok ? off : 0u));
    return ok ? t : make_uint4(0u, 0u, 0u, 0u);
}
__device__ __forceinline__ uint2 ldg8u(const char* base, unsigned off, bool ok) {
    const uint2 t = *reinterpret_cast<const uint2*>(base + (ok ? off : 0u));
    return ok ? t : make_uint2(0u, 0u);
}
__device__ __forceinline__ float4 ldg16f(const char* base, unsigned off, bool ok) {
    const float4 t = *reinterpret_cast<const float4*>(base + (ok ? off : 0u));
    return ok ? t : make_float4(0.f, 0.f, 0.f, 0.f);
}

template <int TM, int TN, int R>
struct TwCfg {
    static constexpr int BM = 16 * TM, BN = 16 * TN, KB = 64;
    static constexpr int IMG = (BM + BN) * KB * 2;
    static constexpr int RED = 3 * TM * TN * 4 * 64 * 4;
    static constexpr int BYTES = (R * IMG > RED) ? R * IMG : RED;
};

template <int TM, int TN, bool TB, int EPI_, bool AF32, int R>
__global__ __launch_bounds__(THREADS) void gemm_bf16tw_kernel(Args a)
{
    using Cfg = TwCfg<TM, TN, R>;
    constexpr int BM = Cfg::BM, BN = Cfg::BN, KB = Cfg::KB;
    extern __shared__ __attribute__((aligned(16))) unsigned char Lds[];
    unsigned short* ImgA = reinterpret_cast<unsigned short*>(Lds);
    unsigned short* ImgB = ImgA + R * BM * KB;
    float* Red = reinterpret_cast<float*>(Lds);

    if ((int)blockIdx.z < a.job_on) {
        const long plane = (long)gridDim.x * gridDim.y;
        air_step_job_run(a.job, blockIdx.z * plane + (long)blockIdx.y * gridDim.x + blockIdx.x, plane * a.job_on);
        return;
    }
    const int nslab = (int)gridDim.z - a.job_on;
    const int zslab = (int)blockIdx.z - a.job_on;
    const int tid = threadIdx.x, lane = tid & 63, wave = tid >> 6;
    int tile_m, tile_n;
    xcd_tile(tile_m, tile_n);
    constexpr bool QUAD = EPI_ == EPI_LSTM_FWD_Q || EPI_ == AIR_EPI_LSTM_FWD0;
    const int m0 = tile_m * BM, n0 = QUAD ? tile_n * 4 : tile_n * BN / TN * (a.gstride == 16 ? TN : 1);
    const int kbeg = zslab * a.kslab;
    const int kend = min(a.K, kbeg + a.kslab);

    AIR_STAMP(56);
    f32x4 acc[TM][TN];
#pragma unroll
    for (int i = 0; i < TM; ++i)
#pragma unroll
        for (int j = 0; j < TN; ++j) acc[i][j] = f32x4{0.f, 0.f, 0.f, 0.f};

    Pre<TM, TN> pre;

    const char* Ab = AF32 ? reinterpret_cast<const char*>(a.A) : reinterpret_cast<const char*>(a.A16);
    const bool pnl = !TB && a.B16p != nullptr;
    const char* Bb = reinterpret_cast<const char*>(pnl ? a.B16p : a.B16);
    const unsigned pK16 = (unsigned)a.K * 16u;
    constexpr int TA_N = AF32 ? (R * BM * 16 + THREADS - 1) / THREADS : (R * BM * 8 + THREADS - 1) / THREADS;
    constexpr int TBK_N = (R * BN * 8 + THREADS - 1) / THREADS;
    constexpr int TBN_N = (R * KB * (BN / 8) + THREADS - 1) / THREADS;
    constexpr int TBQ_N = (R * KB * 4 + THREADS - 1) / THREADS;
    const bool quad16 = EPI_ == AIR_EPI_LSTM_FWD0 && pnl;
    constexpr int TBQ16_N = (TBQ_N + 1) / 2;
    uint4 va[AF32 ? 1 : TA_N];
    float4 vaf[AF32 ? TA_N : 1];
    uint4 vb[QUAD ? 1 : (TB ? TBK_N : TBN_N)];
    uint2 vq[QUAD ? 2 * TBQ16_N : 1];
    const bool twin_out = AF32 && EPI_ == AIR_EPI_LSTM_FWD0 && a.C16 != nullptr && tile_n == 0;
    const int ldt = (a.K + 7) & ~7;

    auto issue_loads = [&](int kr) __attribute__((always_inline)) {
        if (AF32) {
#pragma unroll
            for (int i = 0; i < TA_N; ++i) {
                const int u = tid + THREADS * i;
                const int c = u / (BM * 16), row = (u / 16) % BM, hh = u & 15;
                const int gm = m0 + row, gk = kr + c * KB + hh * 4;
                const bool ok = (u < R * BM * 16) && gm < a.M && gk < kend;
                vaf[i] = ldg16f(Ab, ((unsigned)gm * (unsigned)a.lda + (unsigned)gk) * 4u, ok);
            }
        } else {
#pragma unroll
            for (int i = 0; i < TA_N; ++i) {
                const int u = tid + THREADS * i;
                const int c = u / (BM * 8), row = (u / 8) % BM, g = u & 7;
                const int gm = m0 + row, gk = kr + c * KB + g * 8;
                const bool ok = (u < R * BM * 8) && gm < a.M && gk < kend;
                va[i] = ldg16u(Ab, ((unsigned)gm * (unsigned)a.lda + (unsigned)gk) * 2u, ok);
            }
        }
        if (QUAD && quad16) {
#pragma unroll
            for (int i = 0; i < TBQ16_N; ++i) {
                const int t = tid + THREADS * i;
                const int gk = kr + (t >> 1);
                const bool ok = (t < R * KB * 2) && n0 < a.gwidth && gk < kend;
                const uint4 v = ldg16u(Bb, ((unsigned)(n0 >> 2) * pK16 + (unsigned)kr * 16u) * 2u + (unsigned)t * 16u, ok);
                vq[2 * i] = make_uint2(v.x, v.y); vq[2 * i + 1] = make_uint2(v.z, v.w);
            }
        } else if (QUAD) {
#pragma unroll
            for (int i = 0; i < TBQ_N; ++i) {
                const int t = tid + THREADS * i;
                const int c = t / (KB * 4), k = (t >> 2) % KB, gate = t & 3;
                const int gn = gate * a.gstride + n0, gk = kr + c * KB + k;
                const bool ok = (t < R * KB * 4) && n0 < a.gwidth && gk < kend;
                const unsigned off = pnl ? (unsigned)(n0 >> 2) * pK16 + (unsigned)gk * 16u + (unsigned)gate * 4u
                                         : (unsigned)gk * (unsigned)a.ldb + (unsigned)gn;
                vq[i] = ldg8u(Bb, off * 2u, ok);
            }
        } else if (TB) {
#pragma unroll
            for (int i = 0; i < TBK_N; ++i) {
                const int u = tid + THREADS * i;
                const int c = u / (BN * 8), col = (u / 8) % BN, g = u & 7;
                const int j = col >> 4, cc = col & 15;
                const int gn = n0 + j * a.gstride + cc, cg = n0 + cc + (a.gstride == 16 ? j * 16 : 0);
                const int gk = kr + c * KB + g * 8;
                const bool ok = (u < R * BN * 8) && cg < a.gwidth && gn < a.N && gk < kend;
                vb[i] = ldg16u(Bb, ((unsigned)gn * (unsigned)a.ldb + (unsigned)gk) * 2u, ok);
            }
        } else {
#pragma unroll
            for (int i = 0; i < TBN_N; ++i) {
                const int t = tid + THREADS * i;
                const int c = t / (KB * (BN / 8)), k = (t / (BN / 8)) % KB, h = t % (BN / 8);
                const int col = h * 8, j = col >> 4, cc = col & 15;
                const int gn = n0 + j * a.gstride + cc, cg = n0 + cc + (a.gstride == 16 ? j * 16 : 0);
                const int gk = kr + c * KB + k;
                const bool ok = (t < R * KB * (BN / 8)) && cg < a.gwidth && gn < a.N && gk < kend;
                const unsigned off = pnl ? (unsigned)(gn >> 4) * pK16 + (unsigned)gk * 16u + (unsigned)(gn & 15)
                                         : (unsigned)gk * (unsigned)a.ldb + (unsigned)gn;
                vb[i] = ldg16u(Bb, off * 2u, ok);
            }
        }
    };
    auto store_images = [&](int kr) __attribute__((always_inline)) {
        if (AF32) {
#pragma unroll
            for (int i = 0; i < TA_N; ++i) {
                const int u = tid + THREADS * i;
                const int c = u / (BM * 16), row = (u / 16) % BM, hh = u & 15;
                uint2 w;
                w.x = air_pack_bf16(vaf[i].x, vaf[i].y); w.y = air_pack_bf16(vaf[i].z, vaf[i].w);
                if (u < R * BM * 16)
                    *reinterpret_cast<uint2*>(&ImgA[(c * BM + row) * KB + (((hh >> 1) ^ (row & 7)) << 3) + (hh & 1) * 4]) = w;
                if (twin_out) {
                    const int gm = m0 + row, gk = kr + c * KB + hh * 4;
                    if (u < R * BM * 16 && gm < a.M && gk < ldt)
                        *reinterpret_cast<uint2*>(&a.C16[(size_t)gm * ldt + gk]) = w;
                }
            }
        } else {
#pragma unroll
            for (int i = 0; i < TA_N; ++i) {
                const int u = tid + THREADS * i;
                const int c = u / (BM * 8), row = (u / 8) % BM, g = u & 7;
                if (u < R * BM * 8) *reinterpret_cast<uint4*>(&ImgA[(c * BM + row) * KB + ((g ^ (row & 7)) << 3)]) = va[i];
            }
        }
        if (QUAD && quad16) {
#pragma unroll
            for (int i = 0; i < TBQ16_N; ++i) {
                const int t = tid + THREADS * i;
                if (t < R * KB * 2)
                    *reinterpret_cast<uint4*>(&ImgB[t * 8]) = make_uint4(vq[2 * i].x, vq[2 * i].y, vq[2 * i + 1].x, vq[2 * i + 1].y);
            }
        } else if (QUAD) {
#pragma unroll
            for (int i = 0; i < TBQ_N; ++i) {
                const int t = tid + THREADS * i;
                if (t < R * KB * 4) *reinterpret_cast<uint2*>(&ImgB[t * 4]) = vq[i];
            }
        } else if (TB) {
#pragma unroll
            for (int i = 0; i < TBK_N; ++i) {
                const int u = tid + THREADS * i;
                const int c = u / (BN * 8), col = (u / 8) % BN, g = u & 7;
                if (u < R * BN * 8) *reinterpret_cast<uint4*>(&ImgB[(c * BN + col) * KB + ((g ^ (col & 7)) << 3)]) = vb[i];
            }
        } else {
#pragma unroll
            for (int i = 0; i < TBN_N; ++i) {
                const int t = tid + THREADS * i;
                if (t < R * KB * (BN / 8)) *reinterpret_cast<uint4*>(&ImgB[t * 8]) = vb[i];
            }
        }
    };

    issue_loads(kbeg);
    if (nslab == 1) epilogue_prefetch<TM, TN, EPI_>(a, pre, m0, n0, lane, wave);
    AIR_STAMP(57);
    for (int kr = kbeg; kr < kend; kr += R * KB) {
        if (kr > kbeg) __syncthreads();
        store_images(kr);
        if (kr + R * KB < kend) issue_loads(kr + R * KB);
        __syncthreads();
        AIR_STAMP(58);
        const int cfirst = (wave - ((kr - kbeg) / KB)) & 3;
#pragma unroll
        for (int cc = 0; cc < (R + 3) / 4; ++cc) {
            const int c = cfirst + 4 * cc;
            if (c < R && kr + c * KB < kend) {
#pragma unroll
                for (int ks = 0; ks < 2; ++ks) {
                    const int slot = ks * 4 + (lane >> 4);
                    bf16x8 av[TM], bv[TN];
#pragma unroll
                    for (int i = 0; i < TM; ++i) {
                        const int row = i * 16 + (lane & 15);
                        av[i] = *reinterpret_cast<const bf16x8*>(&ImgA[(c * BM + row) * KB + ((slot ^ (row & 7)) << 3)]);
                    }
                    if (TB) {
#pragma unroll
                        for (int j = 0; j < TN; ++j) {
                            const int col = j * 16 + (lane & 15);
                            bv[j] = *reinterpret_cast<const bf16x8*>(&ImgB[(c * BN + col) * KB + ((slot ^ (col & 7)) << 3)]);
                        }
                    } else {
                        const int il = lane & 15;
                        const unsigned short* blk = &ImgB[(c * KB + ks * 32 + (lane >> 4) * 8 + (il >> 2)) * BN + (il & 3) * 4];
#pragma unroll
                        for (int j = 0; j < TN; ++j) {
                            typedef __attribute__((address_space(3))) s16x4 lds_s16x4;
                            const s16x4 lo = __builtin_amdgcn_ds_read_tr16_b64_v4i16((lds_s16x4*)(blk + j * 16));
                            const s16x4 hi = __builtin_amdgcn_ds_read_tr16_b64_v4i16((lds_s16x4*)(blk + j * 16 + 4 * BN));
                            bv[j] = bf16x8{lo.x, lo.y, lo.z, lo.w, hi.x, hi.y, hi.z, hi.w};
                        }
                    }
#pragma unroll
                    for (int i = 0; i < TM; ++i)
#pragma unroll
                        for (int j = 0; j < TN; ++j)
                            acc[i][j] = __builtin_amdgcn_mfma_f32_16x16x32_bf16(av[i], bv[j], acc[i][j], 0, 0, 0);
                }
            }
        }
    }
    AIR_STAMP(59);
    __syncthreads();
    reduce_waves<TM, TN>(acc, Red, lane, wave);
    AIR_STAMP(60);
    if (nslab > 1) {
        float* Cz = a.C + (size_t)zslab * a.slab_stride;
        for (int t = wave; t < TM * TN; t += 4) {
            const int i = t / TN, j = t % TN;
#pragma unroll
            for (int q = 0; q < 4; ++q) {
                const int m = m0 + i * 16 + (lane >> 4) * 4 + q;
                const int n = n0 + j * 16 + (lane & 15);
                if (m < a.M && n < a.N) Cz[(size_t)m * a.ldc + n] = Red[(t * 4 + q) * 64 + lane];
            }
        }
        return;
    }
    epilogue<TM, TN, EPI_>(a, pre, Red, m0, n0, lane, wave);
    AIR_STAMP(61);
}


template <int BN>
__global__ __launch_bounds__(THREADS) void gemm_xw_tp_kernel(Args a)
{
    constexpr int BM = 64, KB = 64, D = 4;
    constexpr int NJ = BN / 32;
    constexpr int PPR = BN / 8, RPP = THREADS / PPR, NBP = KB / RPP;
    __shared__ __attribute__((aligned(16))) unsigned short ImgA[2][BM * KB];
    __shared__ __attribute__((aligned(16))) unsigned short ImgB[2][KB * BN];
    const int nz = (int)gridDim.z - a.job_on;
    if ((int)blockIdx.z >= nz) {
        const long plane = (long)gridDim.x * gridDim.y;
        air_step_job_run(a.job, ((int)blockIdx.z - nz) * plane + (long)blockIdx.y * gridDim.x + blockIdx.x, plane * a.job_on);
        return;
    }
    const int tid = threadIdx.x, lane = tid & 63, wave = tid >> 6;
    int tile_m = blockIdx.y, tile_n = blockIdx.x, zslab = (int)blockIdx.z;
    {
        const int nx = gridDim.x, ny = gridDim.y, pairs = ny * nz;
        const int lin = (zslab * ny + (int)blockIdx.y) * nx + (int)blockIdx.x;
        const int xcd = lin & 7, slot = lin >> 3;
        if (a.i1 == 0 && (nz & 7) == 0) {
            zslab = xcd + 8 * (slot / (nx * ny));
            const int rem = slot % (nx * ny);
            tile_n = rem % nx; tile_m = rem / nx;
        } else if ((pairs & 7) == 0) {
            const int pair = xcd + 8 * (slot / nx);
            tile_n = slot % nx; tile_m = pair % ny; zslab = pair / ny;
        }
    }
    const int m0 = tile_m * BM, n0 = tile_n * BN;
    const int kbeg = zslab * a.kslab, kend = min(a.K, kbeg + a.kslab);
    const int wm = (wave >> 1) * 32, wn = (wave & 1) * (BN / 2);

    f32x4 acc[2][NJ];
#pragma unroll
    for (int i = 0; i < 2; ++i)
#pragma unroll
        for (int j = 0; j < NJ; ++j) acc[i][j] = f32x4{0.f, 0.f, 0.f, 0.f};

    const int ar = tid >> 4, ah = tid & 15, bk = tid / PPR, bh = tid % PPR;
    const float* pa = a.A + (size_t)(m0 + ar) * a.lda + ah * 4;
    const unsigned short* pb = a.B16 + (size_t)bk * a.ldb + n0 + bh * 8;
    const unsigned la = ar * KB + (((ah >> 1) ^ (ar & 7)) << 3) + (ah & 1) * 4;
    typedef float f32v4 __attribute__((ext_vector_type(4)));
    typedef unsigned u32v4 __attribute__((ext_vector_type(4)));
    f32v4 va[D][4];
    u32v4 vb[D][NBP];
    auto load_stage = [&](auto dc, int k0) __attribute__((always_inline)) {
        constexpr int d = decltype(dc)::value;
#pragma unroll
        for (int i = 0; i < 4; ++i) va[d][i] = *reinterpret_cast<const f32v4*>(pa + (size_t)(16 * i) * a.lda + k0);
#pragma unroll
        for (int i = 0; i < NBP; ++i) vb[d][i] = *reinterpret_cast<const u32v4*>(pb + (size_t)(k0 + RPP * i) * a.ldb);
    };
    int buf = 0;
    auto stage = [&](auto dc, int k0) __attribute__((always_inline)) {
        constexpr int d = decltype(dc)::value;
        if (k0 >= kend) return;
#pragma unroll
        for (int i = 0; i < 4; ++i) {
            uint2 w;
            w.x = air_pack_bf16(va[d][i].x, va[d][i].y); w.y = air_pack_bf16(va[d][i].z, va[d][i].w);
            *reinterpret_cast<uint2*>(&ImgA[buf][la + 16 * i * KB]) = w;
        }
#pragma unroll
        for (int i = 0; i < NBP; ++i) *reinterpret_cast<u32v4*>(&ImgB[buf][(bk + RPP * i) * BN + bh * 8]) = vb[d][i];
        if (k0 + D * KB < kend) load_stage(dc, k0 + D * KB);
        __syncthreads();
#pragma unroll
        for (int ks = 0; ks < 2; ++ks) {
            const int slot = ks * 4 + (lane >> 4), il = lane & 15;
            bf16x8 av[2], bv[NJ];
#pragma unroll
            for (int i = 0; i < 2; ++i) {
                const int row = wm + i * 16 + il;
                av[i] = *reinterpret_cast<const bf16x8*>(&ImgA[buf][row * KB + ((slot ^ (row & 7)) << 3)]);
            }
            const unsigned short* blk = &ImgB[buf][(ks * 32 + (lane >> 4) * 8 + (il >> 2)) * BN + wn + (il & 3) * 4];
#pragma unroll
            for (int j = 0; j < NJ; ++j) {
                typedef __attribute__((address_space(3))) s16x4 lds_s16x4;
                const s16x4 lo = __builtin_amdgcn_ds_read_tr16_b64_v4i16((lds_s16x4*)(blk + j * 16));
                const s16x4 hi = __builtin_amdgcn_ds_read_tr16_b64_v4i16((lds_s16x4*)(blk + j * 16 + 4 * BN));
                bv[j] = bf16x8{lo.x, lo.y, lo.z, lo.w, hi.x, hi.y, hi.z, hi.w};
            }
#pragma unroll
            for (int i = 0; i < 2; ++i)
#pragma unroll
                for (int j = 0; j < NJ; ++j)
                    acc[i][j] = __builtin_amdgcn_mfma_f32_16x16x32_bf16(av[i], bv[j], acc[i][j], 0, 0, 0);
        }
        buf ^= 1;
    };
    using I0 = std::integral_constant<int, 0>; using I1 = std::integral_constant<int, 1>;
    using I2 = std::integral_constant<int, 2>; using I3 = std::integral_constant<int, 3>;
    static_assert(D == 4, "ring depth");
    if (kbeg < kend) load_stage(I0{}, kbeg);
    if (kbeg + KB < kend) load_stage(I1{}, kbeg + KB);
    if (kbeg + 2 * KB < kend) load_stage(I2{}, kbeg + 2 * KB);
    if (kbeg + 3 * KB < kend) load_stage(I3{}, kbeg + 3 * KB);
    for (int kb = kbeg; kb < kend; kb += D * KB) {
        stage(I0{}, kb); stage(I1{}, kb + KB); stage(I2{}, kb + 2 * KB); stage(I3{}, kb + 3 * KB);
    }
    float* Cz = a.C + (size_t)zslab * a.slab_stride;
#pragma unroll
    for (int i = 0; i < 2; ++i)
#pragma unroll
        for (int j = 0; j < NJ; ++j)
#pragma unroll
            for (int q = 0; q < 4; ++q)
                Cz[(size_t)(m0 + wm + i * 16 + (lane >> 4) * 4 + q) * a.ldc + n0 + wn + j * 16 + (lane & 15)] = acc[i][j][q];
}

template <int R>
__global__ __launch_bounds__(THREADS) void gemm_xwx_glds_kernel(Args a)
{
    using Cfg = TwCfg<1, 1, R>;
    constexpr int BM = 16, BN = 16, KB = 64;
    constexpr int EPI_ = AIR_EPI_LSTM_FWD0;
    extern __shared__ __attribute__((aligned(16))) unsigned char Lds[];
    unsigned short* ImgA = reinterpret_cast<unsigned short*>(Lds);
    unsigned short* ImgB = ImgA + R * BM * KB;
    float* Red = reinterpret_cast<float*>(Lds);
    typedef __attribute__((address_space(3))) unsigned char lds_u8;
    typedef const __attribute__((address_space(1))) unsigned char glb_u8;

    if ((int)blockIdx.z < a.job_on) {
        const long plane = (long)gridDim.x * gridDim.y;
        air_step_job_run(a.job, blockIdx.z * plane + (long)blockIdx.y * gridDim.x + blockIdx.x, plane * a.job_on);
        return;
    }
    const int tid = threadIdx.x, lane = tid & 63, wave = tid >> 6;
    int tile_m, tile_n;
    xcd_tile(tile_m, tile_n);
    const int m0 = tile_m * BM, n0 = tile_n * 4;
    const int kbeg = 0, kend = a.K;

    f32x4 acc[1][1];
    acc[0][0] = f32x4{0.f, 0.f, 0.f, 0.f};
    Pre<1, 1> pre;

    const char* Ab = reinterpret_cast<const char*>(a.A16);
    const char* Bb = reinterpret_cast<const char*>(a.B16p) + (size_t)(n0 >> 2) * (size_t)a.K * 32u;
    constexpr int TA_N = R * BM * 8 / THREADS, TB_N = R * KB * 2 / THREADS;
    static_assert((R * BM * 8) % THREADS == 0 && (R * KB * 2) % THREADS == 0, "whole passes of 16-byte pieces");
    lds_u8* const lA = (lds_u8*)Lds;
    lds_u8* const lB = lA + R * BM * KB * 2;
    const uint4 zero4 = make_uint4(0u, 0u, 0u, 0u);
    const int arow = (tid >> 3) & 15, asg = (tid & 7) ^ (arow & 7);
    const int ka = (tid >> 7) * KB + asg * 8, kb = tid >> 1;
    const bool arow_ok = m0 + arow < a.M;
    const int lim_a = arow_ok ? kend : 0, lim_b = n0 < a.gwidth ? kend : 0;
    const char* const pa = Ab + ((size_t)(arow_ok ? m0 + arow : 0) * (size_t)a.lda + (size_t)ka) * 2u;
    const char* const pb = Bb + tid * 16;
    const int wbase = __builtin_amdgcn_readfirstlane(wave) * 1024;

    auto fill_images = [&](int kr) __attribute__((always_inline)) {
#pragma unroll
        for (int i = 0; i < TA_N; ++i)
            if (__builtin_expect(!(kr + 2 * KB * i + ka < lim_a), 0)) *reinterpret_cast<uint4*>(&ImgA[(tid + THREADS * i) * 8]) = zero4;
#pragma unroll
        for (int i = 0; i < TB_N; ++i)
            if (__builtin_expect(!(kr + 2 * KB * i + kb < lim_b), 0)) *reinterpret_cast<uint4*>(&ImgB[(tid + THREADS * i) * 8]) = zero4;
#pragma unroll
        for (int i = 0; i < TA_N; ++i)
            if (__builtin_expect(kr + 2 * KB * i + ka < lim_a, 1))
                __builtin_amdgcn_global_load_lds((glb_u8*)(pa + (size_t)(kr + 2 * KB * i) * 2u), lA + wbase + THREADS * 16 * i, 16, 0, 0);
#pragma unroll
        for (int i = 0; i < TB_N; ++i)
            if (__builtin_expect(kr + 2 * KB * i + kb < lim_b, 1))
                __builtin_amdgcn_global_load_lds((glb_u8*)(pb + (size_t)(kr + 2 * KB * i) * 32u), lB + wbase + THREADS * 16 * i, 16, 0, 0);
    };

    AIR_STAMP(56);
    fill_images(kbeg);
    epilogue_prefetch<1, 1, EPI_>(a, pre, m0, n0, lane, wave);
    AIR_STAMP(57);
    for (int kr = kbeg; kr < kend; kr += R * KB) {
        if (kr > kbeg) { __syncthreads(); fill_images(kr); }
        __syncthreads();
        AIR_STAMP(58);
        const int cfirst = (wave - ((kr - kbeg) / KB)) & 3;
#pragma unroll
        for (int cc = 0; cc < (R + 3) / 4; ++cc) {
            const int c = cfirst + 4 * cc;
            if (c < R && kr + c * KB < kend) {
#pragma unroll
                for (int ks = 0; ks < 2; ++ks) {
                    const int slot = ks * 4 + (lane >> 4);
                    const int row = lane & 15;
                    const bf16x8 av = *reinterpret_cast<const bf16x8*>(&ImgA[(c * BM + row) * KB + ((slot ^ (row & 7)) << 3)]);
                    const int il = lane & 15;
                    const unsigned short* blk = &ImgB[(c * KB + ks * 32 + (lane >> 4) * 8 + (il >> 2)) * BN + (il & 3) * 4];
                    typedef __attribute__((address_space(3))) s16x4 lds_s16x4;
                    const s16x4 lo = __builtin_amdgcn_ds_read_tr16_b64_v4i16((lds_s16x4*)(blk));
                    const s16x4 hi = __builtin_amdgcn_ds_read_tr16_b64_v4i16((lds_s16x4*)(blk + 4 * BN));
                    const bf16x8 bv = bf16x8{lo.x, lo.y, lo.z, lo.w, hi.x, hi.y, hi.z, hi.w};
                    acc[0][0] = __builtin_amdgcn_mfma_f32_16x16x32_bf16(av, bv, acc[0][0], 0, 0, 0);
                }
            }
        }
        if (R >= 40) break;
    }
    AIR_STAMP(59);
    __syncthreads();
    reduce_waves<1, 1>(acc, Red, lane, wave);
    AIR_STAMP(60);
    epilogue<1, 1, EPI_>(a, pre, Red, m0, n0, lane, wave);
    AIR_STAMP(61);
}

#define TW(TM_, TN_, TB_, EPI__, AF_, R_)                                                                               \
    {{BF16TW, TM_, TN_, false, TB_, EPI__, AF_, R_}, reinterpret_cast<const void*>(&gemm_bf16tw_kernel<TM_, TN_, TB_, EPI__, AF_, R_>), \
     TwCfg<TM_, TN_, R_>::BYTES}
#define GLDS(R_) {{XWX_GLDS, 1, 1, false, false, AIR_EPI_LSTM_FWD0, false, R_}, reinterpret_cast<const void*>(&gemm_xwx_glds_kernel<R_>), TwCfg<1, 1, R_>::BYTES}
#define TP(BN_) {{XW_TP, 8, 4, false, false, AIR_EPI_GENERIC, false, BN_}, reinterpret_cast<const void*>(&gemm_xw_tp_kernel<BN_>), 0}
const Kern TWIN_KERNELS[] = {
    TW(1, 1, false, AIR_EPI_LSTM_FWD0, true, 16), TW(1, 1, false, AIR_EPI_LSTM_FWD0, true, 40),
    TW(1, 1, false, AIR_EPI_LSTM_FWD0, false, 16), TW(1, 1, false, AIR_EPI_LSTM_FWD0, false, 40), GLDS(16), GLDS(40),
    TW(1, 1, false, AIR_EPI_GENERIC, false, 4), TW(1, 1, false, AIR_EPI_GENERIC, false, 8), TW(1, 1, false, AIR_EPI_GENERIC, false, 16),
    TW(1, 1, true, AIR_EPI_GENERIC, false, 4), TW(1, 1, true, AIR_EPI_GENERIC, false, 8), TW(1, 1, true, AIR_EPI_GENERIC, false, 16),
    TW(1, 1, true, AIR_EPI_LSTM_BWD, false, 4), TW(1, 1, true, AIR_EPI_LSTM_BWD, false, 8), TW(1, 1, true, AIR_EPI_LSTM_BWD, false, 16),
    TW(1, 1, true, AIR_EPI_LSTM_BWD_TAIL, false, 4), TW(1, 1, true, AIR_EPI_LSTM_BWD_TAIL, false, 8), TW(1, 1, true, AIR_EPI_LSTM_BWD_TAIL, false, 16),
    TW(1, 1, false, EPI_LSTM_FWD_Q, false, 4),
    TW(2, 2, false, AIR_EPI_GENERIC, true, 8), TW(2, 2, false, AIR_EPI_GENERIC, false, 4), TW(2, 2, false, AIR_EPI_GENERIC, false, 8),
    TW(2, 2, true, AIR_EPI_GENERIC, false, 4), TW(2, 2, true, AIR_EPI_GENERIC, false, 8),
    TW(4, 2, false, AIR_EPI_GENERIC, true, 4), TW(4, 2, false, AIR_EPI_GENERIC, false, 4),
    TW(4, 4, false, AIR_EPI_GENERIC, true, 4), TW(4, 4, false, AIR_EPI_GENERIC, false, 4),
    TP(64), TP(128)};
#undef TW
#undef GLDS
#undef TP

}

const Kern* airg::twin_kernels(int& n) {
    n = (int)(sizeof(TWIN_KERNELS) / sizeof(TWIN_KERNELS[0]));
    return TWIN_KERNELS;
}

namespace {

__global__ __launch_bounds__(256) void bf16_twin_kernel(const float* __restrict__ src, unsigned short* __restrict__ dst, long n) {
    const long n4 = n / 4;
    for (long i = (long)blockIdx.x * 256 + threadIdx.x; i < n4; i += (long)gridDim.x * 256) {
        const float4 v = reinterpret_cast<const float4*>(src)[i];
        reinterpret_cast<uint2*>(dst)[i] = make_uint2(air_pack_bf16(v.x, v.y), air_pack_bf16(v.z, v.w));
    }
    if (blockIdx.x == 0 && threadIdx.x < (int)(n - n4 * 4)) dst[n4 * 4 + threadIdx.x] = air_bf16_of(src[n4 * 4 + threadIdx.x]);
}

}

extern "C" int air_bf16_twin(const float* src, uint16_t* dst, int64_t n, void* stream) {
    if (!src || !dst || n <= 0) return AIR_EINVAL;
    if (((reinterpret_cast<uintptr_t>(src) & 15) != 0) || ((reinterpret_cast<uintptr_t>(dst) & 7) != 0)) return AIR_EALIGN;
    long blocks = (n / 4 + 255) / 256;
    blocks = blocks < 1 ? 1 : (blocks > 2048 ? 2048 : blocks);
    hipLaunchKernelGGL(bf16_twin_kernel, dim3((unsigned)blocks), dim3(256), 0, air_stream(stream), src, dst, (long)n);
    AIR_CHECK_LAUNCH();
    return 0;
}
```

tf-attend-infer-repeat_amd/csrc/air_gemm_common.h:

```cpp
#pragma once
#include "air_common.h"
#include "air_philox.h"
#include <type_traits>

namespace airg {

typedef float f32x4 __attribute__((ext_vector_type(4)));
typedef short bf16x8 __attribute__((ext_vector_type(8)));

constexpr int THREADS = 256;
constexpr int EPI_LSTM_FWD_Q = 100;

__device__ __forceinline__ unsigned short f32_to_bf16_rne(float f) {
    unsigned int u = __float_as_uint(f);
    if ((u & 0x7fffffffu) > 0x7f800000u) return (unsigned short)((u >> 16) | 0x40);
    u += 0x7fffu + ((u >> 16) & 1u);
    return (unsigned short)(u >> 16);
}

struct Args {
    const float* A; const float* B; float* C;
    int M, N, K, lda, ldb, ldc;
    int gstride, gwidth;
    int kslab; long slab_stride;
    const float* bias; const float* addend; const float* aux;
    int ldadd, ldaux, add_slabs; long add_slab_stride;
    float aux_scale;
    int act, actgrad, accumulate, epi;
    const float* p0; const float* p1; const float* p2; const float* p3; const float* p4;
    float* q0; float* q1; float* q2; float* q3;
    int i0, i1;
    const unsigned short* A16; const unsigned short* B16;
    unsigned short* C16; unsigned short* q0_16; unsigned short* q2_16;
    const unsigned short* B16p;
    int job_on; AirStepJob job;
};

template <int TM, int TN>
struct Pre {
    static constexpr int NG = TM * TN;
    float bias[NG], add[NG], aux[NG];
    float f[40];
};

template <int TM, int TN, int EPI>
__device__ __forceinline__ void epilogue_prefetch(const Args& a, Pre<TM, TN>& pre, int m0, int n0, int lane, int wave) {
    const int E = EPI < 0 ? a.epi : EPI;
    const float* const safe = a.A;
    if (E == AIR_EPI_GENERIC) {
#pragma unroll
        for (int k = 0; k < TM * TN; ++k) {
            const int it = wave + 4 * k;
            const int i = it / (TN * 4), j = (it >> 2) % TN, q = it & 3;
            const int m = m0 + i * 16 + (lane >> 4) * 4 + q;
            const int n = n0 + j * 16 + (lane & 15);
            const bool ok = m < a.M && n < a.N;
            const bool hb = ok && a.bias, ha = ok && a.addend && a.add_slabs == 1, hx = ok && a.aux;
            pre.bias[k] = *(hb ? a.bias + n : safe);
            pre.add[k] = *(ha ? a.addend + (size_t)m * a.ldadd + n : safe);
            pre.aux[k] = *(hx ? a.aux + (size_t)m * a.ldaux + n : safe);
        }
        return;
    }
    const int q = wave;
    const int m = m0 + (lane >> 4) * 4 + q;
    const int u = n0 + (lane & 15);
    const bool ok = (m < a.M) && (u < a.gwidth);
    auto fetch = [&](bool have, const float* p, size_t off) __attribute__((always_inline)) { return *(have ? p + off : safe); };
    if (E == AIR_EPI_LSTM_FWD) {
        const int R = a.gwidth;
#pragma unroll
        for (int j = 0; j < 4; ++j) {
            const int n = u + j * R;
#pragma unroll
            for (int k = 0; k < 8; ++k)
                pre.f[j * 8 + k] = fetch(ok && k < a.add_slabs, a.addend, k * a.add_slab_stride + (size_t)m * a.ldadd + n);
            pre.f[32 + j] = fetch(ok && a.bias, a.bias, n);
        }
        pre.f[36] = fetch(ok, a.p0, (size_t)m * R + u);
    } else if (E == EPI_LSTM_FWD_Q) {
        const int R = a.gwidth, mm = m0 + (lane >> 2), uu = n0 + (lane & 3);
        const bool okq = mm < a.M && uu < R;
#pragma unroll
        for (int i = 0; i < 37; ++i) pre.f[i] = 0.0f;
        if (wave == 0) {
            const size_t base = (size_t)(okq ? mm : 0) * a.ldadd + (okq ? uu : 0);
            if (a.add_slabs == 4) {
#pragma unroll
                for (int k = 0; k < 4; ++k)
#pragma unroll
                    for (int j = 0; j < 4; ++j) pre.f[j * 8 + k] = a.addend[k * a.add_slab_stride + base + (size_t)j * R];
            } else if (a.add_slabs == 1) {
#pragma unroll
                for (int j = 0; j < 4; ++j) pre.f[j * 8] = a.addend[base + (size_t)j * R];
            } else {
#pragma unroll
                for (int k = 0; k < 8; ++k)
#pragma unroll
                    for (int j = 0; j < 4; ++j)
                        pre.f[j * 8 + k] = fetch(k < a.add_slabs, a.addend, k * a.add_slab_stride + base + (size_t)j * R);
            }
            if (a.bias) {
#pragma unroll
                for (int j = 0; j < 4; ++j) pre.f[32 + j] = a.bias[(okq ? uu : 0) + j * R];
            }
            pre.f[36] = a.p0[(size_t)(okq ? mm : 0) * R + (okq ? uu : 0)];
        }
    } else if (E == AIR_EPI_LSTM_FWD0) {
        const int R = a.gwidth, uu = n0 + (lane & 3);
#pragma unroll
        for (int j = 0; j < 4; ++j) pre.f[j] = fetch(a.bias && uu < R, a.bias, j * R + uu);
    } else if (E == AIR_EPI_REPARAM_FWD) {
        const int Z = a.gwidth;
        pre.f[0] = fetch(ok && a.bias, a.bias, u);
        pre.f[1] = fetch(ok && a.bias, a.bias, Z + u);
        pre.f[2] = fetch(ok, a.p0, (size_t)m * Z + u);
    } else if (E == AIR_EPI_REPARAM_BWD) {
        const int Z = a.gwidth;
        pre.f[0] = fetch(ok, a.p0, (size_t)m * 2 * Z + u);
        pre.f[1] = fetch(ok, a.p0, (size_t)m * 2 * Z + Z + u);
        pre.f[2] = fetch(ok, a.p1, (size_t)m * Z + u);
        pre.f[3] = fetch(ok, a.p2, (size_t)m * AIR_ATT_STRIDE + AIR_ATT_MASK);
        pre.f[4] = a.p3[AIR_DYN_GRAD_SCALE]; pre.f[5] = a.p3[AIR_DYN_VAE_PV]; pre.f[6] = a.p3[AIR_DYN_VAE_PM];
    } else if (E == AIR_EPI_LSTM_BWD || E == AIR_EPI_LSTM_BWD_TAIL) {
        const int R = a.gwidth;
        const int mm = m - (E == AIR_EPI_LSTM_BWD_TAIL ? a.i0 : 0);
        const bool okk = ok && mm >= 0;
        const size_t idx = (size_t)(okk ? mm : 0) * R + u;
#pragma unroll
        for (int j = 0; j < 4; ++j) pre.f[j] = fetch(okk, a.p0, (size_t)(okk ? mm : 0) * 4 * R + j * R + u);
        pre.f[4] = fetch(okk, a.p1, idx);
        pre.f[5] = fetch(okk, a.p2, idx);
        pre.f[6] = fetch(okk && a.p3, a.p3, idx);
        pre.f[7] = fetch(okk && a.addend, a.addend, (size_t)m * a.ldadd + u);
    }
}

template <int TM, int TN, int EPI>
__device__ __forceinline__ void epilogue(const Args& a, const Pre<TM, TN>& pre, const float* Red,
                                         int m0, int n0, int lane, int wave) {
    const int E = EPI < 0 ? a.epi : EPI;
    if (E == AIR_EPI_GENERIC) {
#pragma unroll
        for (int k = 0; k < TM * TN; ++k) {
            const int it = wave + 4 * k;
            const int i = it / (TN * 4), j = (it >> 2) % TN, q = it & 3;
            const int m = m0 + i * 16 + (lane >> 4) * 4 + q;
            const int n = n0 + j * 16 + (lane & 15);
            if (m >= a.M || n >= a.N) continue;
            float v = Red[((i * TN + j) * 4 + q) * 64 + lane];
            if (a.bias) v += pre.bias[k];
            if (a.addend) {
                if (a.add_slabs == 1) v += pre.add[k];
                else for (int sl = 0; sl < a.add_slabs; ++sl) v += a.addend[sl * a.add_slab_stride + (size_t)m * a.ldadd + n];
            }
            if (a.act == AIR_ACT_RELU) v = fmaxf(v, 0.0f);
            else if (a.act == AIR_ACT_SOFTPLUS) v = air_softplus(v);
            else if (a.act == AIR_ACT_SIGMOID_NOISE) v = air_sigmoid(v + pre.aux[k] * a.aux_scale);
            if (a.actgrad == AIR_GRAD_RELU) v = (pre.aux[k] > 0.0f) ? v : 0.0f;
            else if (a.actgrad == AIR_GRAD_SOFTPLUS) v = v * (1.0f - expf(-pre.aux[k]));
            float* c = a.C + (size_t)m * a.ldc + n;
            if (a.accumulate) v += *c;
            *c = v;
            if (a.C16) a.C16[(size_t)m * a.ldc + n] = air_bf16_of(v);
        }
        return;
    }
    if (E == EPI_LSTM_FWD_Q) {
        if (wave == 0) {
            const int R = a.gwidth, r = lane >> 2, m = m0 + r, u = n0 + (lane & 3);
            if (m < a.M && u < R) {
                float g[4];
#pragma unroll
                for (int j = 0; j < 4; ++j) {
                    float s = Red[(r & 3) * 64 + (r >> 2) * 16 + j * 4 + (lane & 3)];
#pragma unroll
                    for (int k = 0; k < 8; ++k) s += (k < a.add_slabs) ? pre.f[j * 8 + k] : 0.0f;
                    if (a.bias) s += pre.f[32 + j];
                    g[j] = s;
                }
                const float si = air_sigmoid(g[0]), tj = tanhf(g[1]);
                const float sf = air_sigmoid(g[2] + 1.0f), so = air_sigmoid(g[3]);
                const float cn = pre.f[36] * sf + si * tj;
                float* ac = a.q0 + (size_t)m * 4 * R;
                ac[u] = si; ac[R + u] = tj; ac[2 * R + u] = sf; ac[3 * R + u] = so;
                a.q1[(size_t)m * R + u] = cn;
                const float hn = tanhf(cn) * so;
                a.q2[(size_t)m * R + u] = hn;
                if (a.q2_16) a.q2_16[(size_t)m * R + u] = air_bf16_of(hn);
            }
        }
        return;
    }
    if (E == AIR_EPI_LSTM_FWD0) {
        const int R = a.gwidth;
        {
            const int m = m0 + (lane >> 4) * 4 + wave, col = lane & 15, u = n0 + (col & 3);
            if (m < a.M && u < R) a.C[(size_t)m * a.ldc + (col >> 2) * R + u] = Red[wave * 64 + lane];
        }
        if (wave == 0) {
            const int r = lane >> 2, m = m0 + r, u = n0 + (lane & 3);
            if (m < a.M && u < R) {
                float g[4];
#pragma unroll
                for (int j = 0; j < 4; ++j) {
                    float s = Red[(r & 3) * 64 + (r >> 2) * 16 + j * 4 + (lane & 3)];
                    if (a.bias) s += pre.f[j];
                    g[j] = s;
                }
                const float si = air_sigmoid(g[0]), tj = tanhf(g[1]);
                const float sf = air_sigmoid(g[2] + 1.0f), so = air_sigmoid(g[3]);
                const float cn = 0.0f * sf + si * tj;
                float* ac = a.q0 + (size_t)m * 4 * R;
                ac[u] = si; ac[R + u] = tj; ac[2 * R + u] = sf; ac[3 * R + u] = so;
                a.q1[(size_t)m * R + u] = cn;
                const float hn = tanhf(cn) * so;
                a.q2[(size_t)m * R + u] = hn;
                if (a.q2_16) a.q2_16[(size_t)m * R + u] = air_bf16_of(hn);
            }
        }
        return;
    }
    for (int it = wave; it < TM * 4; it += 4) {
        const int i = it >> 2, q = it & 3;
        const int m = m0 + i * 16 + (lane >> 4) * 4 + q;
        const int u = n0 + (lane & 15);
        if (m >= a.M || u >= a.gwidth) continue;
        float v[TN];
#pragma unroll
        for (int j = 0; j < TN; ++j) v[j] = Red[((i * TN + j) * 4 + q) * 64 + lane];
        if (E == AIR_EPI_LSTM_FWD) {
            if (TN == 4 && TM == 1) {
                const int R = a.gwidth;
                float g[4];
#pragma unroll
                for (int j = 0; j < 4; ++j) {
                    float s = v[j % TN];
#pragma unroll
                    for (int k = 0; k < 8; ++k) s += (k < a.add_slabs) ? pre.f[j * 8 + k] : 0.0f;
                    if (a.bias) s += pre.f[32 + j];
                    g[j] = s;
                }
                const float si = air_sigmoid(g[0]), tj = tanhf(g[1]);
                const float sf = air_sigmoid(g[2] + 1.0f), so = air_sigmoid(g[3]);
                const float cn = pre.f[36] * sf + si * tj;
                float* ac = a.q0 + (size_t)m * 4 * R;
                ac[u] = si; ac[R + u] = tj; ac[2 * R + u] = sf; ac[3 * R + u] = so;
                a.q1[(size_t)m * R + u] = cn;
                const float hn = tanhf(cn) * so;
                a.q2[(size_t)m * R + u] = hn;
                if (a.q2_16) a.q2_16[(size_t)m * R + u] = air_bf16_of(hn);
            }
        } else if (E == AIR_EPI_REPARAM_FWD) {
            if (TN == 2) {
                const int Z = a.gwidth;
                const float mean = v[0] + (a.bias ? pre.f[0] : 0.0f);
                const float lv = v[1 % TN] + (a.bias ? pre.f[1] : 0.0f);
                a.C[(size_t)m * a.ldc + u] = mean;
                a.C[(size_t)m * a.ldc + Z + u] = lv;
                const float zv = mean + pre.f[2] * sqrtf(expf(lv));
                a.q0[(size_t)m * Z + u] = zv;
                if (a.q0_16) a.q0_16[(size_t)m * Z + u] = air_bf16_of(zv);
            }
        } else if (E == AIR_EPI_LSTM_BWD || E == AIR_EPI_LSTM_BWD_TAIL) {
            if (TM == 1) {
                const int R = a.gwidth;
                const bool tail = E == AIR_EPI_LSTM_BWD_TAIL;
                const float addv = a.addend ? pre.f[7] : 0.0f;
                if (tail && m < a.i0) { a.C[(size_t)m * a.ldc + u] = v[0] + addv; continue; }
                const int mrow = tail ? m - a.i0 : m;
                const bool accumulate = tail ? false : (a.i0 != 0);
                const float dhv = v[0] + addv;
                const float si = pre.f[0], tj = pre.f[1], sf = pre.f[2], so = pre.f[3];
                const size_t idx = (size_t)mrow * R + u;
                const float tc = tanhf(pre.f[5]);
                const float dc = (a.p3 ? pre.f[6] : 0.0f) + dhv * so * (1.0f - tc * tc);
                const float dgi = dc * tj * si * (1.0f - si);
                const float dgj = dc * si * (1.0f - tj * tj);
                const float dgf = dc * pre.f[4] * sf * (1.0f - sf);
                const float dgo = dhv * tc * so * (1.0f - so);
                float* dg = a.q0 + (size_t)mrow * 4 * R;
                dg[u] = dgi; dg[R + u] = dgj; dg[2 * R + u] = dgf; dg[3 * R + u] = dgo;
                if (a.q0_16) {
                    unsigned short* dgb = a.q0_16 + (size_t)mrow * 4 * R;
                    dgb[u] = air_bf16_of(dgi); dgb[R + u] = air_bf16_of(dgj); dgb[2 * R + u] = air_bf16_of(dgf); dgb[3 * R + u] = air_bf16_of(dgo);
                }
                a.q1[idx] = dc * sf;
                if (a.q2) {
                    float* ds = a.q2 + (size_t)mrow * 4 * R;
                    float s0 = dgi, s1 = dgj, s2 = dgf, s3 = dgo;
                    if (accumulate) { s0 = ds[u] + dgi; s1 = ds[R + u] + dgj; s2 = ds[2 * R + u] + dgf; s3 = ds[3 * R + u] + dgo; }
                    ds[u] = s0; ds[R + u] = s1; ds[2 * R + u] = s2; ds[3 * R + u] = s3;
                    if (a.q2_16) {
                        unsigned short* dsb = a.q2_16 + (size_t)mrow * 4 * R;
                        dsb[u] = air_bf16_of(s0); dsb[R + u] = air_bf16_of(s1); dsb[2 * R + u] = air_bf16_of(s2); dsb[3 * R + u] = air_bf16_of(s3);
                    }
                }
            }
        } else if (E == AIR_EPI_REPARAM_BWD) {
            const int Z = a.gwidth;
            const float klg = pre.f[3] * pre.f[4];
            const float pv = pre.f[5], pm = pre.f[6];
            const float var = expf(pre.f[1]);
            const float sd = sqrtf(var);
            const float d = v[0];
            const float dmean = d + klg * (pre.f[0] - pm) / pv;
            const float dlv = d * pre.f[2] * 0.5f * sd + klg * 0.5f * (var / pv - 1.0f);
            a.C[(size_t)m * a.ldc + u] = dmean;
            a.C[(size_t)m * a.ldc + Z + u] = dlv;
            if (a.C16) { a.C16[(size_t)m * a.ldc + u] = air_bf16_of(dmean); a.C16[(size_t)m * a.ldc + Z + u] = air_bf16_of(dlv); }
        }
    }
}

template <int TM, int TN>
__device__ __forceinline__ void reduce_waves(f32x4 (&acc)[TM][TN], float* Red, int lane, int wave) {
    constexpr int RS = TM * TN * 4 * 64;
    if (wave > 0) {
        float* r = Red + (wave - 1) * RS;
#pragma unroll
        for (int i = 0; i < TM; ++i)
#pragma unroll
            for (int j = 0; j < TN; ++j)
#pragma unroll
                for (int q = 0; q < 4; ++q) r[((i * TN + j) * 4 + q) * 64 + lane] = acc[i][j][q];
    }
    __syncthreads();
    if (wave == 0) {
#pragma unroll
        for (int i = 0; i < TM; ++i)
#pragma unroll
            for (int j = 0; j < TN; ++j)
#pragma unroll
                for (int q = 0; q < 4; ++q) {
                    const int o = ((i * TN + j) * 4 + q) * 64 + lane;
                    float v = acc[i][j][q];
#pragma unroll
                    for (int w = 0; w < 3; ++w) v += Red[w * RS + o];
                    Red[o] = v;
                }
    }
    __syncthreads();
}

__device__ __forceinline__ void xcd_tile(int& tile_m, int& tile_n) {
    const int nx = gridDim.x, ny = gridDim.y, nwg = nx * ny;
    const int bid = blockIdx.y * nx + blockIdx.x;
    const int q = nwg >> 3, r = nwg & 7, xcd = bid & 7;
    const int swz = (xcd < r ? xcd * (q + 1) : r * (q + 1) + (xcd - r) * q) + (bid >> 3);
    tile_m = swz % ny;
    tile_n = swz / ny;
}

__host__ __device__ __forceinline__ bool aligned16(const void* p) { return (reinterpret_cast<uintptr_t>(p) & 15) == 0; }

enum Family { F32, BF16, F32V2, BF16V2, BF16TW, XWX_GLDS, XW_TP };
struct Inst {
    int family, tm, tn;
    bool ta, tb;
    int epi;
    bool af32;
    int r;
};
inline bool operator==(const Inst& x, const Inst& y) {
    return x.family == y.family && x.tm == y.tm && x.tn == y.tn && x.ta == y.ta && x.tb == y.tb && x.epi == y.epi &&
           x.af32 == y.af32 && x.r == y.r;
}
struct Kern { Inst inst; const void* fn; int lds; };
struct Plan {
    Inst inst;
    const void* fn; int lds;
    dim3 grid;
    Args args;
};
int plan_gemm(const air_gemm_t* g, const Args& filled, Plan& p);
const Kern* twin_kernels(int& n);

}
```

Baseline: 374,700 images/sec.

## Stage bf16 GEMM tiles with per-wave direct-to-LDS loads, dropping block barriers

Adds a wave-owned staging path for the bf16 tiled GEMM. Each wave fills only the LDS images it later consumes, using global_load_lds, and waits with s_waitcnt instead of block-wide __syncthreads. The existing quad-panel DMA kernel is converted to the same scheme. An explicit `grouped` flag replaces the `gstride==16` test, since grouped layouts could otherwise collide with a stride of 16. A debug LDS-fill entry point is also added. The risk is correctness: it relies on each wave reading only its own images, otherwise there are cross-wave LDS races.

```diff
diff --git a/include/air_hip.h b/include/air_hip.h
--- a/include/air_hip.h
+++ b/include/air_hip.h
@@ -108,6 +108,8 @@
 
 int air_bf16_twin(const float* src, uint16_t* dst, int64_t n, void* stream);
 
+int air_debug_lds_fill(uint32_t pattern, int bytes, int workgroups, void* stream);
+
 typedef struct {
     int64_t src_off, dst_off;
     int32_t K, N, gates, exclusive;
diff --git a/tf-attend-infer-repeat_amd/air/_hip.py b/tf-attend-infer-repeat_amd/air/_hip.py
--- a/tf-attend-infer-repeat_amd/air/_hip.py
+++ b/tf-attend-infer-repeat_amd/air/_hip.py
@@ -147,6 +147,7 @@
     "air_gemm_kernel_name": (C.c_int, [C.POINTER(Gemm), C.c_char_p, C.c_int]),
     "air_gemm_slabs": (C.c_int, [C.c_int, C.c_int]),
     "air_bf16_twin": (C.c_int, [_p, _p, C.c_int64, _p]),
+    "air_debug_lds_fill": (C.c_int, [C.c_uint32, C.c_int, C.c_int, _p]),
     "air_panel_shadow": (C.c_int, [_p, _p, C.POINTER(Panel), C.c_int, _p]),
     "air_adam_clip_step_panels": (C.c_int, [_p, _p, _p, _p, C.c_int64, _p, C.c_int, _p, _p, _f, _f, _f, _f, _p,
                                             C.POINTER(Panel), C.c_int, _p, _p, _p]),
diff --git a/tf-attend-infer-repeat_amd/csrc/air_gemm.hip b/tf-attend-infer-repeat_amd/csrc/air_gemm.hip
--- a/tf-attend-infer-repeat_amd/csrc/air_gemm.hip
+++ b/tf-attend-infer-repeat_amd/csrc/air_gemm.hip
@@ -34,7 +34,7 @@
     const int tid = threadIdx.x, lane = tid & 63, wave = tid >> 6;
     int tile_m, tile_n;
     xcd_tile(tile_m, tile_n);
-    const int m0 = tile_m * BM, n0 = tile_n * BN / TN * (a.gstride == 16 ? TN : 1);
+    const int m0 = tile_m * BM, n0 = tile_n * BN / TN * (!a.grouped ? TN : 1);
     const int kbeg = zslab * a.kslab;
     const int kend = min(a.K, kbeg + a.kslab);
 
@@ -119,7 +119,7 @@
             const int it = tid + THREADS * i;
             const int k = it / NQ, q4 = it % NQ;
             const int j = q4 >> 2, c = (q4 & 3) * 4;
-            const int cg = n0 + c + (a.gstride == 16 ? j * 16 : 0);
+            const int cg = n0 + c + (!a.grouped ? j * 16 : 0);
             const int gn = n0 + j * a.gstride + c, gk = k0 + k;
             if (gk < kend) {
                 const float* src = a.B + (size_t)gk * a.ldb + gn;
@@ -235,7 +235,7 @@
     const int tid = threadIdx.x, lane = tid & 63, wave = tid >> 6;
     int tile_m, tile_n;
     xcd_tile(tile_m, tile_n);
-    const int m0 = tile_m * BM, n0 = tile_n * BN / TN * (a.gstride == 16 ? TN : 1);
+    const int m0 = tile_m * BM, n0 = tile_n * BN / TN * (!a.grouped ? TN : 1);
     const int kbeg = zslab * a.kslab;
     const int kend = min(a.K, kbeg + a.kslab);
 
@@ -257,7 +257,7 @@
             int n, k;
             if (TB) { n = idx / BK; k = idx % BK; } else { k = idx / BN; n = idx % BN; }
             const int j = n >> 4, c = n & 15;
-            const int cg = n0 + c + (a.gstride == 16 ? j * 16 : 0);
+            const int cg = n0 + c + (!a.grouped ? j * 16 : 0);
             const int gn = n0 + j * a.gstride + c, gk = k0 + k;
             float v = 0.0f;
             if (cg < a.gwidth && gn < a.N && gk < kend)
@@ -376,7 +376,7 @@
     const int tid = threadIdx.x, lane = tid & 63, wave = tid >> 6;
     int tile_m, tile_n;
     xcd_tile(tile_m, tile_n);
-    const int m0 = tile_m * BM, n0 = EPI_ == AIR_EPI_LSTM_FWD0 ? tile_n * 4 : tile_n * BN / TN * (a.gstride == 16 ? TN : 1);
+    const int m0 = tile_m * BM, n0 = EPI_ == AIR_EPI_LSTM_FWD0 ? tile_n * 4 : tile_n * BN / TN * (!a.grouped ? TN : 1);
     const int kbeg = zslab * a.kslab;
     const int kend = min(a.K, kbeg + a.kslab);
 
@@ -418,7 +418,7 @@
                 const int u = tid + THREADS * i;
                 const int c = u / (BN * 16), col = (u / 16) % BN, hh = u & 15;
                 const int j = col >> 4, cc = col & 15;
-                const int gn = n0 + j * a.gstride + cc, cg = n0 + cc + (a.gstride == 16 ? j * 16 : 0);
+                const int gn = n0 + j * a.gstride + cc, cg = n0 + cc + (!a.grouped ? j * 16 : 0);
                 const int gk = kr + c * KB + hh * 4;
                 const bool okr = (u < R * BN * 16) && cg < a.gwidth && gn < a.N;
                 const unsigned off = ((unsigned)gn * (unsigned)a.ldb + (unsigned)gk) * 4u;
@@ -431,7 +431,7 @@
                 const int c = t / (BN * 2), q = (t / 8) % (BN / 4), g = t & 7;
                 const int col = q * 4, j = col >> 4, cc = col & 15;
                 const int gn = EPI_ == AIR_EPI_LSTM_FWD0 ? n0 + q * a.gstride : n0 + j * a.gstride + cc;
-                const int cg = EPI_ == AIR_EPI_LSTM_FWD0 ? n0 : n0 + cc + (a.gstride == 16 ? j * 16 : 0);
+                const int cg = EPI_ == AIR_EPI_LSTM_FWD0 ? n0 : n0 + cc + (!a.grouped ? j * 16 : 0);
                 const int gk = kr + c * KB + g * 8;
                 const bool okc = (t < R * BN * 2) && cg < a.gwidth && gn < a.N;
                 const bool okh = okc && cg + 2 < a.gwidth && gn + 2 < a.N;
@@ -584,7 +584,7 @@
     int tile_m, tile_n;
     xcd_tile(tile_m, tile_n);
     constexpr bool QUADF = EPI_ == AIR_EPI_LSTM_FWD0 || EPI_ == EPI_LSTM_FWD_Q;
-    const int m0 = tile_m * BM, n0 = QUADF ? tile_n * 4 : tile_n * BN / TN * (a.gstride == 16 ? TN : 1);
+    const int m0 = tile_m * BM, n0 = QUADF ? tile_n * 4 : tile_n * BN / TN * (!a.grouped ? TN : 1);
     const int kbeg = zslab * a.kslab;
     const int kend = min(a.K, kbeg + a.kslab);
 
@@ -627,7 +627,7 @@
                 const int t = tid + THREADS * i;
                 const int c = t / (BN * 8), col = (t / 8) % BN, g = t & 7;
                 const int j = col >> 4, cc = col & 15;
-                const int gn = n0 + j * a.gstride + cc, cg = n0 + cc + (a.gstride == 16 ? j * 16 : 0);
+                const int gn = n0 + j * a.gstride + cc, cg = n0 + cc + (!a.grouped ? j * 16 : 0);
                 const int gk = kr + c * KB + g * 8;
                 const bool okr = (t < R * BN * 8) && cg < a.gwidth && gn < a.N;
                 const unsigned off = ((unsigned)gn * (unsigned)a.ldb + (unsigned)gk) * 4u;
@@ -641,7 +641,7 @@
                 const int c = t / (BN * 2), q = (t / 8) % (BN / 4), g = t & 7;
                 const int col = q * 4, j = col >> 4, cc = col & 15;
                 const int gn = QUADF ? n0 + q * a.gstride : n0 + j * a.gstride + cc;
-                const int cg = QUADF ? n0 : n0 + cc + (a.gstride == 16 ? j * 16 : 0);
+                const int cg = QUADF ? n0 : n0 + cc + (!a.grouped ? j * 16 : 0);
                 const int gk = kr + c * KB + g * 8;
                 const bool okc = (t < R * BN * 2) && cg < a.gwidth && gn < a.N;
                 const bool okh = okc && cg + 2 < a.gwidth && gn + 2 < a.N;
@@ -851,6 +851,17 @@
     return 0;
 }
 
+bool tw_wave_dma(const Inst& i, const Args& a) {
+    if (i.family != BF16TW || i.af32 || i.epi == AIR_EPI_LSTM_FWD0 || (i.r & 3)) return false;
+    const bool pnl = !i.tb && a.B16p != nullptr;
+    if (!aligned16(a.A16) || (a.lda & 7)) return false;
+    if (pnl ? !aligned16(a.B16p) : (!aligned16(a.B16) || (a.ldb & 7))) return false;
+    if (i.epi == EPI_LSTM_FWD_Q && !pnl) return false;
+    if ((a.K < a.kslab ? a.K : a.kslab) < 256) return false;
+    if (i.tm == 1 && i.tn == 1 && i.epi == AIR_EPI_GENERIC && (i.tb || i.r == 8)) return false;
+    return true;
+}
+
 int xw_tp_ok(const Args& a, int precision, bool ta, bool tb, int ksplit) {
     auto al16 = [](const void* p) { return (reinterpret_cast<uintptr_t>(p) & 15) == 0; };
     if (precision != 1 || ta || tb || !a.B16 || a.epi != AIR_EPI_GENERIC || ksplit <= 1) return AIR_EINVAL;
@@ -884,7 +895,7 @@
         int tm, tn;
         resolve_tile(g, tm, tn);
         if (!find_kernel(Inst{F32, tm, tn, false, false, -1, false, 0})) return AIR_EINVAL;
-        const bool grouped = a.gstride != 16;
+        const bool grouped = a.grouped != 0;
         const int ncols = grouped ? a.gwidth : a.N;
         const int tile_cols = a.epi == AIR_EPI_LSTM_FWD0 ? 4 : (grouped ? 16 : 16 * tn);
         p.grid = dim3((ncols + tile_cols - 1) / tile_cols, (a.M + 16 * tm - 1) / (16 * tm), 1);
@@ -910,6 +921,7 @@
         }
     }
     p.grid.z = (a.K + a.kslab - 1) / a.kslab + a.job_on;
+    a.wave_dma = tw_wave_dma(p.inst, a);
     const Kern* k = find_kernel(p.inst);
     if (!k) return AIR_EINVAL;
     if ((size_t)k->lds > AIR_LDS_LIMIT) return AIR_ELIMIT;
@@ -983,7 +995,7 @@
     if (g->aux && g->ldaux < g->N) return AIR_EINVAL;
     a.A = g->A; a.B = g->B; a.C = g->C;
     a.M = g->M; a.N = g->N; a.K = g->K; a.lda = g->lda; a.ldb = g->ldb; a.ldc = g->ldc;
-    a.gstride = 16; a.gwidth = g->N;
+    a.gstride = 16; a.gwidth = g->N; a.grouped = 0;
     a.kslab = g->K; a.slab_stride = 0;
     a.bias = g->bias; a.addend = g->addend; a.aux = g->aux;
     a.ldadd = g->ldadd; a.ldaux = g->ldaux;
@@ -997,6 +1009,7 @@
     a.A16 = g->A16; a.B16 = g->B16; a.C16 = g->C16; a.q0_16 = g->q0_16; a.q2_16 = g->q2_16;
     a.B16p = (g->precision == 1 && !g->transA && !g->transB) ? g->B16p : nullptr;
     a.job_on = 0;
+    a.wave_dma = 0;
     if (g->step_job) {
         const air_step_job_t& j = *g->step_job;
         if (!j.dyn || !j.istate || j.nsched < 0 || j.nsched > THREADS || (j.nsched > 0 && !j.sched)) return AIR_EINVAL;
@@ -1010,13 +1023,13 @@
     switch (g->epi) {
         case AIR_EPI_LSTM_FWD:
             if (g->transA || g->transB || (g->N & 3) || !g->p0 || !g->q0 || !g->q1 || !g->q2) return AIR_EINVAL;
-            a.gstride = g->N / 4; a.gwidth = g->N / 4; break;
+            a.gstride = g->N / 4; a.gwidth = g->N / 4; a.grouped = 1; break;
         case AIR_EPI_LSTM_FWD0:
             if (g->transA || g->transB || (g->N & 15) || g->addend || !g->q0 || !g->q1 || !g->q2) return AIR_EINVAL;
-            a.gstride = g->N / 4; a.gwidth = g->N / 4; break;
+            a.gstride = g->N / 4; a.gwidth = g->N / 4; a.grouped = 1; break;
         case AIR_EPI_REPARAM_FWD:
             if (g->transA || g->transB || (g->N & 1) || !g->p0 || !g->q0) return AIR_EINVAL;
-            a.gstride = g->N / 2; a.gwidth = g->N / 2; break;
+            a.gstride = g->N / 2; a.gwidth = g->N / 2; a.grouped = 1; break;
         case AIR_EPI_LSTM_BWD:
             if (!g->p0 || !g->p1 || !g->p2 || !g->q0 || !g->q1) return AIR_EINVAL;
             a.gwidth = g->N; break;
diff --git a/tf-attend-infer-repeat_amd/csrc/air_gemm_bf16.hip b/tf-attend-infer-repeat_amd/csrc/air_gemm_bf16.hip
--- a/tf-attend-infer-repeat_amd/csrc/air_gemm_bf16.hip
+++ b/tf-attend-infer-repeat_amd/csrc/air_gemm_bf16.hip
@@ -23,6 +23,74 @@
     const float4 t = *reinterpret_cast<const float4*>(base + (ok ? off : 0u));
     return ok ? t : make_float4(0.f, 0.f, 0.f, 0.f);
 }
+
+typedef __attribute__((address_space(3))) unsigned char lds_u8;
+typedef const __attribute__((address_space(1))) unsigned char glb_u8;
+
+template <int TM, int TN, bool TB, bool QUAD, int R, class F>
+__device__ __forceinline__ void wave_pieces(const Args& a, const char* Ab, const char* Bb, bool pnl, int m0, int n0,
+                                            int kr, int kend, int lane, int wv, F f)
+{
+    constexpr int BM = 16 * TM, BN = 16 * TN, KB = 64;
+    constexpr unsigned IMGA = BM * KB * 2, IMGB = BN * KB * 2, OFFB = R * IMGA;
+    static_assert(R % 4 == 0, "a wave owns the same images in every round");
+    const int r8 = lane >> 3, sg = (lane & 7) ^ r8;
+    const unsigned pK16 = (unsigned)a.K * 16u;
+#pragma unroll
+    for (int ci = 0; ci < R / 4; ++ci) {
+        const int c = wv + 4 * ci, k0 = kr + c * KB;
+        if (k0 >= kend) break;
+#pragma unroll
+        for (int p = 0; p < 2 * TM; ++p) {
+            const int gm = m0 + p * 8 + r8, gk = k0 + sg * 8;
+            f(gm < a.M && gk < kend, Ab + ((unsigned)gm * (unsigned)a.lda + (unsigned)gk) * 2u, c * IMGA + p * 1024u);
+        }
+        if (QUAD) {
+#pragma unroll
+            for (int p = 0; p < 2; ++p) {
+                const int t = p * 64 + lane, gk = k0 + (t >> 1);
+                f(n0 < a.gwidth && gk < kend, Bb + ((unsigned)(n0 >> 2) * pK16 + (unsigned)k0 * 16u) * 2u + (unsigned)t * 16u,
+                  OFFB + c * IMGB + p * 1024u);
+            }
+        } else if (TB) {
+#pragma unroll
+            for (int p = 0; p < 2 * TN; ++p) {
+                const int col = p * 8 + r8, j = col >> 4, cc = col & 15;
+                const int gn = n0 + j * a.gstride + cc, cg = n0 + cc + (!a.grouped ? j * 16 : 0);
+                const int gk = k0 + sg * 8;
+                f(cg < a.gwidth && gn < a.N && gk < kend, Bb + ((unsigned)gn * (unsigned)a.ldb + (unsigned)gk) * 2u,
+                  OFFB + c * IMGB + p * 1024u);
+            }
+        } else {
+#pragma unroll
+            for (int p = 0; p < 2 * TN; ++p) {
+                const int t = p * 64 + lane, k = t / (BN / 8), h = t % (BN / 8);
+                const int col = h * 8, j = col >> 4, cc = col & 15;
+                const int gn = n0 + j * a.gstride + cc, cg = n0 + cc + (!a.grouped ? j * 16 : 0);
+                const int gk = k0 + k;
+                const unsigned off = pnl ? (unsigned)(gn >> 4) * pK16 + (unsigned)gk * 16u + (unsigned)(gn & 15)
+                                         : (unsigned)gk * (unsigned)a.ldb + (unsigned)gn;
+                f(cg < a.gwidth && gn < a.N && gk < kend, Bb + off * 2u, OFFB + c * IMGB + p * 1024u);
+            }
+        }
+    }
+}
+
+template <int TM, int TN, bool TB, bool QUAD, int R>
+__device__ __forceinline__ void wave_fill(const Args& a, unsigned char* Lds, const char* Ab, const char* Bb, bool pnl,
+                                          int m0, int n0, int kr, int kend, int lane, int wv)
+{
+    wave_pieces<TM, TN, TB, QUAD, R>(a, Ab, Bb, pnl, m0, n0, kr, kend, lane, wv,
+        [&](bool ok, const char*, unsigned off) __attribute__((always_inline)) {
+            if (__builtin_expect(!ok, 0)) *reinterpret_cast<uint4*>(Lds + off + lane * 16) = make_uint4(0u, 0u, 0u, 0u);
+        });
+    wave_pieces<TM, TN, TB, QUAD, R>(a, Ab, Bb, pnl, m0, n0, kr, kend, lane, wv,
+        [&](bool ok, const char* src, unsigned off) __attribute__((always_inline)) {
+            if (__builtin_expect(ok, 1)) __builtin_amdgcn_global_load_lds((glb_u8*)src, (lds_u8*)Lds + off, 16, 0, 0);
+        });
+}
+__device__ __forceinline__ void wave_fills_landed() { asm volatile("s_waitcnt vmcnt(0)" ::: "memory"); }
+__device__ __forceinline__ void wave_reads_returned() { asm volatile("s_waitcnt lgkmcnt(0)" ::: "memory"); }
 
 template <int TM, int TN, int R>
 struct TwCfg {
@@ -53,7 +121,7 @@
     int tile_m, tile_n;
     xcd_tile(tile_m, tile_n);
     constexpr bool QUAD = EPI_ == EPI_LSTM_FWD_Q || EPI_ == AIR_EPI_LSTM_FWD0;
-    const int m0 = tile_m * BM, n0 = QUAD ? tile_n * 4 : tile_n * BN / TN * (a.gstride == 16 ? TN : 1);
+    const int m0 = tile_m * BM, n0 = QUAD ? tile_n * 4 : tile_n * BN / TN * (!a.grouped ? TN : 1);
     const int kbeg = zslab * a.kslab;
     const int kend = min(a.K, kbeg + a.kslab);
 
@@ -129,7 +197,7 @@
                 const int u = tid + THREADS * i;
                 const int c = u / (BN * 8), col = (u / 8) % BN, g = u & 7;
                 const int j = col >> 4, cc = col & 15;
-                const int gn = n0 + j * a.gstride + cc, cg = n0 + cc + (a.gstride == 16 ? j * 16 : 0);
+                const int gn = n0 + j * a.gstride + cc, cg = n0 + cc + (!a.grouped ? j * 16 : 0);
                 const int gk = kr + c * KB + g * 8;
                 const bool ok = (u < R * BN * 8) && cg < a.gwidth && gn < a.N && gk < kend;
                 vb[i] = ldg16u(Bb, ((unsigned)gn * (unsigned)a.ldb + (unsigned)gk) * 2u, ok);
@@ -140,7 +208,7 @@
                 const int t = tid + THREADS * i;
                 const int c = t / (KB * (BN / 8)), k = (t / (BN / 8)) % KB, h = t % (BN / 8);
                 const int col = h * 8, j = col >> 4, cc = col & 15;
-                const int gn = n0 + j * a.gstride + cc, cg = n0 + cc + (a.gstride == 16 ? j * 16 : 0);
+                const int gn = n0 + j * a.gstride + cc, cg = n0 + cc + (!a.grouped ? j * 16 : 0);
                 const int gk = kr + c * KB + k;
                 const bool ok = (t < R * KB * (BN / 8)) && cg < a.gwidth && gn < a.N && gk < kend;
                 const unsigned off = pnl ? (unsigned)(gn >> 4) * pK16 + (unsigned)gk * 16u + (unsigned)(gn & 15)
@@ -202,15 +270,7 @@
         }
     };
 
-    issue_loads(kbeg);
-    if (nslab == 1) epilogue_prefetch<TM, TN, EPI_>(a, pre, m0, n0, lane, wave);
-    AIR_STAMP(57);
-    for (int kr = kbeg; kr < kend; kr += R * KB) {
-        if (kr > kbeg) __syncthreads();
-        store_images(kr);
-        if (kr + R * KB < kend) issue_loads(kr + R * KB);
-        __syncthreads();
-        AIR_STAMP(58);
+    auto mfma_round = [&](int kr) __attribute__((always_inline)) {
         const int cfirst = (wave - ((kr - kbeg) / KB)) & 3;
 #pragma unroll
         for (int cc = 0; cc < (R + 3) / 4; ++cc) {
@@ -249,6 +309,38 @@
                             acc[i][j] = __builtin_amdgcn_mfma_f32_16x16x32_bf16(av[i], bv[j], acc[i][j], 0, 0, 0);
                 }
             }
+        }
+    };
+
+    constexpr bool DMA = !AF32 && EPI_ != AIR_EPI_LSTM_FWD0;
+    bool staged = false;
+    if constexpr (DMA) if (a.wave_dma) {
+        staged = true;
+        const int wv = __builtin_amdgcn_readfirstlane(wave);
+        wave_fill<TM, TN, TB, QUAD, R>(a, Lds, Ab, Bb, pnl, m0, n0, kbeg, kend, lane, wv);
+        if (nslab == 1) epilogue_prefetch<TM, TN, EPI_>(a, pre, m0, n0, lane, wave);
+        AIR_STAMP(57);
+        for (int kr = kbeg; kr < kend; kr += R * KB) {
+            if (kr > kbeg) {
+                wave_reads_returned();
+                wave_fill<TM, TN, TB, QUAD, R>(a, Lds, Ab, Bb, pnl, m0, n0, kr, kend, lane, wv);
+            }
+            wave_fills_landed();
+            AIR_STAMP(58);
+            mfma_round(kr);
+        }
+    }
+    if (!staged) {
+        issue_loads(kbeg);
+        if (nslab == 1) epilogue_prefetch<TM, TN, EPI_>(a, pre, m0, n0, lane, wave);
+        AIR_STAMP(57);
+        for (int kr = kbeg; kr < kend; kr += R * KB) {
+            if (kr > kbeg) __syncthreads();
+            store_images(kr);
+            if (kr + R * KB < kend) issue_loads(kr + R * KB);
+            __syncthreads();
+            AIR_STAMP(58);
+            mfma_round(kr);
         }
     }
     AIR_STAMP(59);
@@ -396,8 +488,6 @@
     unsigned short* ImgA = reinterpret_cast<unsigned short*>(Lds);
     unsigned short* ImgB = ImgA + R * BM * KB;
     float* Red = reinterpret_cast<float*>(Lds);
-    typedef __attribute__((address_space(3))) unsigned char lds_u8;
-    typedef const __attribute__((address_space(1))) unsigned char glb_u8;
 
     if ((int)blockIdx.z < a.job_on) {
         const long plane = (long)gridDim.x * gridDim.y;
@@ -415,44 +505,19 @@
     Pre<1, 1> pre;
 
     const char* Ab = reinterpret_cast<const char*>(a.A16);
-    const char* Bb = reinterpret_cast<const char*>(a.B16p) + (size_t)(n0 >> 2) * (size_t)a.K * 32u;
-    constexpr int TA_N = R * BM * 8 / THREADS, TB_N = R * KB * 2 / THREADS;
-    static_assert((R * BM * 8) % THREADS == 0 && (R * KB * 2) % THREADS == 0, "whole passes of 16-byte pieces");
-    lds_u8* const lA = (lds_u8*)Lds;
-    lds_u8* const lB = lA + R * BM * KB * 2;
-    const uint4 zero4 = make_uint4(0u, 0u, 0u, 0u);
-    const int arow = (tid >> 3) & 15, asg = (tid & 7) ^ (arow & 7);
-    const int ka = (tid >> 7) * KB + asg * 8, kb = tid >> 1;
-    const bool arow_ok = m0 + arow < a.M;
-    const int lim_a = arow_ok ? kend : 0, lim_b = n0 < a.gwidth ? kend : 0;
-    const char* const pa = Ab + ((size_t)(arow_ok ? m0 + arow : 0) * (size_t)a.lda + (size_t)ka) * 2u;
-    const char* const pb = Bb + tid * 16;
-    const int wbase = __builtin_amdgcn_readfirstlane(wave) * 1024;
-
-    auto fill_images = [&](int kr) __attribute__((always_inline)) {
-#pragma unroll
-        for (int i = 0; i < TA_N; ++i)
-            if (__builtin_expect(!(kr + 2 * KB * i + ka < lim_a), 0)) *reinterpret_cast<uint4*>(&ImgA[(tid + THREADS * i) * 8]) = zero4;
-#pragma unroll
-        for (int i = 0; i < TB_N; ++i)
-            if (__builtin_expect(!(kr + 2 * KB * i + kb < lim_b), 0)) *reinterpret_cast<uint4*>(&ImgB[(tid + THREADS * i) * 8]) = zero4;
-#pragma unroll
-        for (int i = 0; i < TA_N; ++i)
-            if (__builtin_expect(kr + 2 * KB * i + ka < lim_a, 1))
-                __builtin_amdgcn_global_load_lds((glb_u8*)(pa + (size_t)(kr + 2 * KB * i) * 2u), lA + wbase + THREADS * 16 * i, 16, 0, 0);
-#pragma unroll
-        for (int i = 0; i < TB_N; ++i)
-            if (__builtin_expect(kr + 2 * KB * i + kb < lim_b, 1))
-                __builtin_amdgcn_global_load_lds((glb_u8*)(pb + (size_t)(kr + 2 * KB * i) * 32u), lB + wbase + THREADS * 16 * i, 16, 0, 0);
-    };
+    const char* Bb = reinterpret_cast<const char*>(a.B16p);
+    const int wv = __builtin_amdgcn_readfirstlane(wave);
 
     AIR_STAMP(56);
-    fill_images(kbeg);
+    wave_fill<1, 1, false, true, R>(a, Lds, Ab, Bb, true, m0, n0, kbeg, kend, lane, wv);
     epilogue_prefetch<1, 1, EPI_>(a, pre, m0, n0, lane, wave);
     AIR_STAMP(57);
     for (int kr = kbeg; kr < kend; kr += R * KB) {
-        if (kr > kbeg) { __syncthreads(); fill_images(kr); }
-        __syncthreads();
+        if (kr > kbeg) {
+            wave_reads_returned();
+            wave_fill<1, 1, false, true, R>(a, Lds, Ab, Bb, true, m0, n0, kr, kend, lane, wv);
+        }
+        wave_fills_landed();
         AIR_STAMP(58);
         const int cfirst = (wave - ((kr - kbeg) / KB)) & 3;
 #pragma unroll
@@ -526,6 +591,28 @@
 
 }
 
+namespace {
+
+__global__ __launch_bounds__(256) void debug_lds_fill_kernel(unsigned pattern, int words, unsigned* sink) {
+    extern __shared__ __attribute__((aligned(16))) unsigned char Lds[];
+    volatile unsigned* w = reinterpret_cast<volatile unsigned*>(Lds);
+    for (int i = threadIdx.x; i < words; i += 256) w[i] = pattern;
+    __syncthreads();
+    if (sink && w[(threadIdx.x * 61) % words] != pattern) *sink = 1u;
+}
+
+}
+
+extern "C" int air_debug_lds_fill(uint32_t pattern, int bytes, int workgroups, void* stream) {
+    if (bytes < 4 || (bytes & 3) || workgroups <= 0 || workgroups > 65535) return AIR_EINVAL;
+    int rc = air_grant_lds(reinterpret_cast<const void*>(&debug_lds_fill_kernel), (size_t)bytes);
+    if (rc) return rc;
+    hipLaunchKernelGGL(debug_lds_fill_kernel, dim3((unsigned)workgroups), dim3(256), (size_t)bytes, air_stream(stream),
+                       (unsigned)pattern, bytes / 4, (unsigned*)nullptr);
+    AIR_CHECK_LAUNCH();
+    return 0;
+}
+
 extern "C" int air_bf16_twin(const float* src, uint16_t* dst, int64_t n, void* stream) {
     if (!src || !dst || n <= 0) return AIR_EINVAL;
     if (((reinterpret_cast<uintptr_t>(src) & 15) != 0) || ((reinterpret_cast<uintptr_t>(dst) & 7) != 0)) return AIR_EALIGN;
diff --git a/tf-attend-infer-repeat_amd/csrc/air_gemm_common.h b/tf-attend-infer-repeat_amd/csrc/air_gemm_common.h
--- a/tf-attend-infer-repeat_amd/csrc/air_gemm_common.h
+++ b/tf-attend-infer-repeat_amd/csrc/air_gemm_common.h
@@ -22,6 +22,7 @@
     const float* A; const float* B; float* C;
     int M, N, K, lda, ldb, ldc;
     int gstride, gwidth;
+    int grouped;
     int kslab; long slab_stride;
     const float* bias; const float* addend; const float* aux;
     int ldadd, ldaux, add_slabs; long add_slab_stride;
@@ -34,6 +35,7 @@
     unsigned short* C16; unsigned short* q0_16; unsigned short* q2_16;
     const unsigned short* B16p;
     int job_on; AirStepJob job;
+    int wave_dma;
 };
 
 template <int TM, int TN>
```

After: 377,400 images/sec, median of 6. About the same (+0.7%).
